# erizmr/SPH_Taichi

Hardware: AMD Instinct MI355X
Metric: WCSPH steps/sec at 1.74 M particles (+ ms/step breakdown sort/neighbour/force) (higher is better)
Workload: dtype f32

## Files before the change

### include/sph_hip.h

```cpp
#ifndef SPH_HIP_H
#define SPH_HIP_H

#include <stddef.h>
#include <stdint.h>

#ifdef __cplusplus
extern "C" {
#endif

#define SPH_ABI_VERSION 6

typedef struct SphContext SphContext;

typedef struct SphParams {
    int32_t n_particles;
    int32_t capacity;
    int32_t grid_num[3];
    int32_t cell_origin[3];
    int32_t n_objects;
    int32_t cold_capacity;
    float grid_size;
    float support_radius;
    float particle_diameter;
    float m_V0;
    float density_0;
    float stiffness;
    float exponent;
    float viscosity;
    float surface_tension;
    float dt;
    float g[3];
    float domain_size[3];
    float padding;
    float wall_hi[3];
    float k_w;
    float k_dw;
    float visc_d_nu;
    float visc_eps;
} SphParams;

enum SphField {
    SPH_F_OBJECT_ID = 0,
    SPH_F_X = 1,
    SPH_F_X_0 = 2,
    SPH_F_V = 3,
    SPH_F_ACCELERATION = 4,
    SPH_F_M_V = 5,
    SPH_F_M = 6,
    SPH_F_DENSITY = 7,
    SPH_F_PRESSURE = 8,
    SPH_F_MATERIAL = 9,
    SPH_F_COLOR = 10,
    SPH_F_IS_DYNAMIC = 11,
    SPH_F_GRID_IDS = 12,
    SPH_F_GRID_PARTICLES_NUM = 13,
    SPH_F_PID = 14,
    SPH_F_RIGID_REST_CM = 15,
    SPH_F_DFSPH_FACTOR = 16,
    SPH_F_DENSITY_ADV = 17,
    SPH_F_COUNT_ = 18
};

enum SphError {
    SPH_OK = 0,
    SPH_E_INVALID = -1,
    SPH_E_NO_DEVICE = -2,
    SPH_E_NOMEM = -3,
    SPH_E_STATE = -4
};

enum SphOption {
    SPH_OPT_GATHER_IMPL = 0,
    SPH_OPT_TIMING = 1,
    SPH_OPT_FUSED_STEP = 2,
    SPH_OPT_BRICK_SHAPE = 3,
    SPH_OPT_NO_DYNAMIC_SOLIDS = 4 ,
    SPH_OPT_DEBUG_ABLATE = 5,
    SPH_OPT_SLAB_DROP_OUTSIDE = 6 ,
    SPH_OPT_UNIFORM_FLUID = 7  ,
    SPH_OPT_UNIFORM_FLUID_STATE = 8 ,
    SPH_OPT_SORT_BY_PID = 9    ,
    SPH_OPT_KERNEL_VARIANT = 10 ,
    SPH_OPT_RIGID_BATCH = 11   ,
    SPH_OPT_DF_RUNAHEAD = 13,
    SPH_OPT_EXACT_MATH = 12    ,
    SPH_OPT_RIGID_SUMS_FROM_X0 = 14,
    SPH_OPT_PURE_FLUID_INSTANCE = 15 ,
    SPH_OPT_BRICK_RECORDS = 16 ,
    SPH_OPT_DF_FUSE_ERROR = 17
};
#define SPH_VAR_GROUPS 1
#define SPH_VAR_MFMA 32
#define SPH_VAR_GAT_LDS 2
#define SPH_VAR_GAT_LDS4 4
#define SPH_VAR_FORCE_BF 8
#define SPH_VAR_DEEP 16

typedef struct SphTimings {
    double sort_ms, neighbour_ms, force_ms, integrate_ms, halo_ms, total_ms;
    int64_t steps;
} SphTimings;

int32_t sph_abi_version(void);
int32_t sph_device_count(void);

int32_t sph_create(const SphParams* params, int32_t device, void* stream, SphContext** out);
int32_t sph_destroy(SphContext* ctx);
const char* sph_last_error(const SphContext* ctx);
int32_t sph_set_option(SphContext* ctx, int32_t option, int32_t value);
int32_t sph_get_option(const SphContext* ctx, int32_t option, int32_t* value);
int32_t sph_set_params(SphContext* ctx, const SphParams* params);
int32_t sph_set_dt(SphContext* ctx, float dt);
int32_t sph_set_particle_count(SphContext* ctx, int32_t n);

int32_t sph_upload(SphContext* ctx, int32_t field, const void* host, size_t bytes);
int32_t sph_download(SphContext* ctx, int32_t field, void* host, size_t bytes);

int32_t sph_update_grid_id(SphContext* ctx);
int32_t sph_prefix_sum(SphContext* ctx);
int32_t sph_counting_sort(SphContext* ctx);
int32_t sph_initialize_particle_system(SphContext* ctx);

int32_t sph_compute_boundary_volume(SphContext* ctx, int32_t dynamic);
int32_t sph_compute_densities(SphContext* ctx);
int32_t sph_compute_non_pressure_forces(SphContext* ctx);
int32_t sph_compute_pressure_forces(SphContext* ctx);
int32_t sph_advect(SphContext* ctx);
int32_t sph_enforce_boundary_3D(SphContext* ctx, int32_t particle_type);
int32_t sph_compute_rigid_rest_cm(SphContext* ctx, int32_t object_id);
int32_t sph_solve_constraints(SphContext* ctx, int32_t object_id, float* R_out);
int32_t sph_compute_com(SphContext* ctx, int32_t object_id, float* cm_out);

int32_t sph_step(SphContext* ctx, int32_t n_steps, const int32_t* dynamic_ids, int32_t n_dynamic);

int32_t sph_sync(SphContext* ctx);
int32_t sph_get_timings(SphContext* ctx, SphTimings* out);
int32_t sph_reset_timings(SphContext* ctx);

typedef struct SphStats {
    int64_t targets;
    int64_t list_entries;
    int32_t max_list;
    int32_t list_overflow_targets;
    int32_t lds_overflow_targets;
    int32_t max_cell_occupancy;
    int32_t nonempty_cells;
    int32_t polar_fallbacks;
} SphStats;
int32_t sph_get_stats(SphContext* ctx, SphStats* out);

#define SPH_RECORD_BYTES 48
int32_t sph_get_particle_count(SphContext* ctx, int32_t* n);
int32_t sph_layer_offsets(SphContext* ctx, const int32_t* layers, int32_t n, int32_t* out);
int32_t sph_layer_offsets_begin(SphContext* ctx, const int32_t* layers, int32_t n);
int32_t sph_layer_offsets_end(SphContext* ctx, int32_t* out, int32_t n);
int32_t sph_select_range(SphContext* ctx, int32_t first, int32_t count);
int32_t sph_truncate(SphContext* ctx, int32_t n);
int32_t sph_pack_range(SphContext* ctx, int32_t first, int32_t count, void* device_dst);
int32_t sph_append_records(SphContext* ctx, const void* device_src, int32_t count);
int32_t sph_set_target_layers(SphContext* ctx, int32_t density_lo, int32_t density_hi, int32_t force_lo, int32_t force_hi);
int32_t sph_slab_set_window(SphContext* ctx, int32_t origin_x, int32_t nx);
int32_t sph_slab_pack(SphContext* ctx, int32_t firstL, int32_t nL, void* dstL, int32_t firstR, int32_t nR, void* dstR);
int32_t sph_slab_advance(SphContext* ctx, int32_t keep_first, int32_t keep_count, const void* srcL, int32_t nL,
                         const void* srcR, int32_t nR, const int32_t* layers, int32_t n_layers, int32_t do_sweeps);
int32_t sph_slab_forces(SphContext* ctx, int32_t bl_lo, int32_t bl_hi, int32_t br_lo, int32_t br_hi,
                        int32_t firstL, int32_t nL, void* dstL, int32_t firstR, int32_t nR, void* dstR);
int32_t sph_slab_wait_pack(SphContext* ctx);
int32_t sph_slab_density(SphContext* ctx);
int32_t sph_sort(SphContext* ctx);
int32_t sph_sweeps(SphContext* ctx);

int32_t sph_rigid_partial_sums(SphContext* ctx, int32_t object_id, int32_t first, int32_t count, double* dev_sums16);
int32_t sph_rigid_apply_sums(SphContext* ctx, int32_t object_id, const double* dev_sums16, int32_t mode);
int32_t sph_upload_rest_positions(SphContext* ctx, const int32_t* pid, const float* x0, int32_t n);

typedef struct SphComm SphComm;
const char* sph_comm_last_error(void);
int32_t sph_comm_available(void);
int32_t sph_comm_unique_id(uint8_t* out128);
int32_t sph_comm_create(SphContext* ctx, const uint8_t* id128, int32_t rank, int32_t world, SphComm** out);
int32_t sph_comm_destroy(SphComm* comm);
int32_t sph_slab_announce(SphContext* ctx, SphComm* comm, int32_t left, int32_t right, int32_t n_to_left, int32_t n_to_right);
int32_t sph_slab_incoming(SphContext* ctx, SphComm* comm, int32_t* n_from_left, int32_t* n_from_right);
int32_t sph_slab_exchange(SphContext* ctx, SphComm* comm, int32_t left, int32_t right, const void* send_left, int32_t n_to_left,
                          const void* send_right, int32_t n_to_right, void* recv_left, int32_t n_from_left, void* recv_right,
                          int32_t n_from_right, int32_t after_packers);
int32_t sph_comm_swap(SphContext* ctx, SphComm* comm, int32_t left, int32_t right, const void* send_left, int64_t bytes_to_left,
                      const void* send_right, int64_t bytes_to_right, void* recv_left, int64_t bytes_from_left, void* recv_right,
                      int64_t bytes_from_right);
int32_t sph_comm_all_reduce(SphContext* ctx, SphComm* comm, void* dev, int32_t n, int32_t dtype);
int32_t sph_comm_sync(SphContext* ctx, SphComm* comm);
int32_t sph_comm_halo_time(SphContext* ctx, SphComm* comm, double* ms, int64_t* exchanges);
int32_t sph_comm_info(SphContext* ctx, SphComm* comm, int32_t* rank, int32_t* world);

typedef struct SphDfsphParams {
    int32_t enable_divergence_solver;
    int32_t m_max_iterations_v;
    int32_t m_max_iterations;
    int32_t fluid_particle_num;
    float m_eps;
    float reserved_;
    double max_error_V;
    double max_error;
} SphDfsphParams;

typedef struct SphDfsphStats {
    int32_t iterations_v;
    int32_t iterations;
    double avg_density_err_v;
    double avg_density_err;
    int64_t total_iterations_v;
    int64_t total_iterations;
    int64_t steps;
} SphDfsphStats;

int32_t sph_dfsph_set_params(SphContext* ctx, const SphDfsphParams* params);
int32_t sph_dfsph_get_stats(SphContext* ctx, SphDfsphStats* out);
int32_t sph_dfsph_compute_densities(SphContext* ctx);
int32_t sph_dfsph_compute_DFSPH_factor(SphContext* ctx);
int32_t sph_dfsph_compute_density_change(SphContext* ctx);
int32_t sph_dfsph_compute_density_adv(SphContext* ctx);
int32_t sph_dfsph_compute_density_error(SphContext* ctx, float offset, float* out);
int32_t sph_dfsph_multiply_time_step(SphContext* ctx, float time_step);
int32_t sph_dfsph_divergence_solver_iteration_kernel(SphContext* ctx);
int32_t sph_dfsph_pressure_solve_iteration_kernel(SphContext* ctx);
int32_t sph_dfsph_divergence_solve(SphContext* ctx);
int32_t sph_dfsph_pressure_solve(SphContext* ctx);
int32_t sph_dfsph_compute_non_pressure_forces(SphContext* ctx);
int32_t sph_dfsph_predict_velocity(SphContext* ctx);
int32_t sph_dfsph_advect(SphContext* ctx);
int32_t sph_dfsph_step(SphContext* ctx, int32_t n_steps, const int32_t* dynamic_ids, int32_t n_dynamic);
int32_t sph_dfsph_compute_density_error_range(SphContext* ctx, float offset, int32_t first, int32_t count, double* out);
int32_t sph_copy_velocity_records(SphContext* ctx, int32_t first, int32_t count, void* device_buf, int32_t to_context);

#define SPH_RENDER_MAX_INVISIBLE 32
typedef struct SphRenderParams {
    int32_t width, height;
    float eye[3], lookat[3], up[3];
    float fov_y_deg;
    float radius;
    float near_plane;
    float light[3];
    float ambient;
    uint8_t background[3], draw_box;
    float box_end[3];
    float box_color[3];
} SphRenderParams;
int32_t sph_render_set_params(SphContext* ctx, const SphRenderParams* params);
int32_t sph_render_set_invisible(SphContext* ctx, const int32_t* object_ids, int32_t n);
int32_t sph_render_frame(SphContext* ctx);
int32_t sph_render_download(SphContext* ctx, uint8_t* rgb, size_t bytes);
int32_t sph_render_download_depth(SphContext* ctx, float* depth, size_t bytes);

#define SPH_MAX_KINEMATIC 8
typedef struct SphKinematicMotion {
    int32_t object_id;
    float pivot[3];
    double lin_vel[3], ang_vel[3], osc_amplitude[3], osc_frequency, osc_phase, start_time, end_time;
} SphKinematicMotion;
typedef struct SphBodyPose {
    int32_t object_id;
    float R[9];
    float pivot[3], origin[3], lin_vel[3], ang_vel[3];
} SphBodyPose;
int32_t sph_kinematic_set(SphContext* ctx, const SphKinematicMotion* motions, int32_t n);
int32_t sph_kinematic_apply(SphContext* ctx, const SphBodyPose* poses, int32_t n);
int32_t sph_get_time(SphContext* ctx, double* t);
int32_t sph_set_time(SphContext* ctx, double t);

#define SPH_DIAG_BLOCKS 1024
#define SPH_DIAG_THREADS 256
#define SPH_DIAG_MAX_OBJECTS 96
typedef struct SphDiagRow {
    int64_t count;
    int64_t fluid_count;
    int64_t moving_count;
    double mass;
    double mx[3];
    double momentum[3];
    double kinetic;
    double v2_max;
    double a2_max;
    float density_min, density_max, pressure_min, pressure_max;
    float lo[3], hi[3];
} SphDiagRow;
int32_t sph_diag_reduce(SphContext* ctx);
int32_t sph_diag_download(SphContext* ctx, SphDiagRow* rows, int32_t n_rows);

#define SPH_COLUMNS_MAX (1 << 20)
#define SPH_COLUMNS_V_SCALE_LOG2 20
typedef struct SphColumnParams {
    int32_t axis;
    int32_t n[2];
    float origin[2], inv_cell[2];
    int32_t object_id;
} SphColumnParams;
typedef struct SphColumnTotals { int64_t selected, binned, outside; } SphColumnTotals;
int32_t sph_columns_reduce(SphContext* ctx, const SphColumnParams* params);
int32_t sph_columns_download(SphContext* ctx, int64_t* count, int64_t* sum_v , float* top, float* bottom,
                             int32_t n_columns, SphColumnTotals* totals);

#define SPH_EXPORT_X        1
#define SPH_EXPORT_V        2
#define SPH_EXPORT_DENSITY  4
#define SPH_EXPORT_PRESSURE 8
#define SPH_EXPORT_MASS     16
#define SPH_EXPORT_ID       32
#define SPH_EXPORT_OBJECT   64
#define SPH_EXPORT_MAX_OBJECTS 32
typedef struct SphExportParams {
    int32_t fields;
    int32_t material;
    int32_t n_objects;
    int32_t object_ids[SPH_EXPORT_MAX_OBJECTS];
    int32_t pid_stride, pid_phase;
    int32_t use_box;
    float box_lo[3], box_hi[3];
} SphExportParams;
typedef struct SphExportInfo { int64_t selected, rows; int32_t row_bytes, duplicate_ids; } SphExportInfo;
int32_t sph_export_select(SphContext* ctx, const SphExportParams* params);
int32_t sph_export_info(SphContext* ctx, SphExportInfo* info);
int32_t sph_export_download(SphContext* ctx, void* host, size_t bytes);

#define SPH_SURFACE_MAX_FILTER_R 16
#define SPH_SURFACE_MAX_ITERATIONS 8
#define SPH_SURFACE_PASSES 6
typedef struct SphSurfaceParams {
    int32_t iterations;
    float filter_radius;
    float depth_range;
    float fluid_color[3];
    float absorb[3];
    float sky[3];
    float f0;
    float specular;
} SphSurfaceParams;
int32_t sph_surface_set_params(SphContext* ctx, const SphSurfaceParams* params);
int32_t sph_surface_frame(SphContext* ctx);
int32_t sph_surface_download(SphContext* ctx, uint8_t* rgb, size_t bytes);
int32_t sph_surface_download_depth(SphContext* ctx, float* depth, size_t bytes);
int32_t sph_surface_download_thickness(SphContext* ctx, float* thickness, size_t bytes);
int32_t sph_surface_frame_timed(SphContext* ctx, float* ms, int32_t n);

#define SPH_FIELD_MAX_OBJECTS 32
enum SphColourField { SPH_FIELD_SPEED = 0, SPH_FIELD_VX, SPH_FIELD_VY, SPH_FIELD_VZ, SPH_FIELD_DENSITY, SPH_FIELD_PRESSURE,
                      SPH_FIELD_X, SPH_FIELD_Y, SPH_FIELD_Z, SPH_FIELD_COUNT_ };
typedef struct SphFieldColour {
    int32_t field;
    int32_t material;
    int32_t n_objects;
    int32_t object_ids[SPH_FIELD_MAX_OBJECTS];
    float lo, hi;
    float axis_origin;
} SphFieldColour;
typedef struct SphFieldRange { float lo, hi; int64_t count, non_finite; } SphFieldRange;
int32_t sph_frame_set_colour(SphContext* ctx, const SphFieldColour* colour, const int32_t* lut);
int32_t sph_field_range(SphContext* ctx, const SphFieldColour* colour, SphFieldRange* out);
int32_t sph_frame_download_field_index(SphContext* ctx, int32_t* index, size_t bytes);

#ifdef __cplusplus
}
#endif
#endif
```

### sph_taichi_amd/_lib.py

```python
from __future__ import annotations

import ctypes as C
import os

from . import build as _build

_F3 = C.c_float * 3
_I3 = C.c_int32 * 3


class SphParams(C.Structure):
    _fields_ = [
        ("n_particles", C.c_int32), ("capacity", C.c_int32), ("grid_num", _I3), ("cell_origin", _I3),
        ("n_objects", C.c_int32), ("cold_capacity", C.c_int32),
        ("grid_size", C.c_float), ("support_radius", C.c_float), ("particle_diameter", C.c_float),
        ("m_V0", C.c_float), ("density_0", C.c_float), ("stiffness", C.c_float), ("exponent", C.c_float),
        ("viscosity", C.c_float), ("surface_tension", C.c_float), ("dt", C.c_float),
        ("g", _F3), ("domain_size", _F3), ("padding", C.c_float), ("wall_hi", _F3),
        ("k_w", C.c_float), ("k_dw", C.c_float), ("visc_d_nu", C.c_float), ("visc_eps", C.c_float),
    ]


class SphTimings(C.Structure):
    _fields_ = [("sort_ms", C.c_double), ("neighbour_ms", C.c_double), ("force_ms", C.c_double),
                ("integrate_ms", C.c_double), ("halo_ms", C.c_double), ("total_ms", C.c_double),
                ("steps", C.c_int64)]


class SphStats(C.Structure):
    _fields_ = [("targets", C.c_int64), ("list_entries", C.c_int64), ("max_list", C.c_int32),
                ("list_overflow_targets", C.c_int32), ("lds_overflow_targets", C.c_int32),
                ("max_cell_occupancy", C.c_int32), ("nonempty_cells", C.c_int32), ("polar_fallbacks", C.c_int32)]


class SphDfsphParams(C.Structure):
    _fields_ = [("enable_divergence_solver", C.c_int32), ("m_max_iterations_v", C.c_int32),
                ("m_max_iterations", C.c_int32), ("fluid_particle_num", C.c_int32), ("m_eps", C.c_float),
                ("reserved_", C.c_float), ("max_error_V", C.c_double), ("max_error", C.c_double)]


class SphDfsphStats(C.Structure):
    _fields_ = [("iterations_v", C.c_int32), ("iterations", C.c_int32), ("avg_density_err_v", C.c_double),
                ("avg_density_err", C.c_double), ("total_iterations_v", C.c_int64), ("total_iterations", C.c_int64),
                ("steps", C.c_int64)]


class SphRenderParams(C.Structure):
    _fields_ = [("width", C.c_int32), ("height", C.c_int32), ("eye", _F3), ("lookat", _F3), ("up", _F3),
                ("fov_y_deg", C.c_float), ("radius", C.c_float), ("near_plane", C.c_float), ("light", _F3),
                ("ambient", C.c_float), ("background", C.c_uint8 * 3), ("draw_box", C.c_uint8),
                ("box_end", _F3), ("box_color", _F3)]


RENDER_MAX_INVISIBLE = 32
_D3 = C.c_double * 3


class SphKinematicMotion(C.Structure):
    _fields_ = [("object_id", C.c_int32), ("pivot", _F3), ("lin_vel", _D3), ("ang_vel", _D3), ("osc_amplitude", _D3),
                ("osc_frequency", C.c_double), ("osc_phase", C.c_double), ("start_time", C.c_double), ("end_time", C.c_double)]


class SphBodyPose(C.Structure):
    _fields_ = [("object_id", C.c_int32), ("R", C.c_float * 9), ("pivot", _F3), ("origin", _F3), ("lin_vel", _F3),
                ("ang_vel", _F3)]


MAX_KINEMATIC = 8


class SphDiagRow(C.Structure):
    _fields_ = [("count", C.c_int64), ("fluid_count", C.c_int64), ("moving_count", C.c_int64), ("mass", C.c_double),
                ("mx", _D3), ("momentum", _D3), ("kinetic", C.c_double), ("v2_max", C.c_double), ("a2_max", C.c_double),
                ("density_min", C.c_float), ("density_max", C.c_float), ("pressure_min", C.c_float),
                ("pressure_max", C.c_float), ("lo", _F3), ("hi", _F3)]


DIAG_BLOCKS, DIAG_THREADS, DIAG_MAX_OBJECTS = 1024, 256, 96

class SphColumnParams(C.Structure):
    _fields_ = [("axis", C.c_int32), ("n", C.c_int32 * 2), ("origin", C.c_float * 2), ("inv_cell", C.c_float * 2),
                ("object_id", C.c_int32)]


class SphColumnTotals(C.Structure):
    _fields_ = [("selected", C.c_int64), ("binned", C.c_int64), ("outside", C.c_int64)]


COLUMNS_MAX, COLUMNS_V_SCALE_LOG2 = 1 << 20, 20

class SphExportParams(C.Structure):
    _fields_ = [("fields", C.c_int32), ("material", C.c_int32), ("n_objects", C.c_int32), ("object_ids", C.c_int32 * 32),
                ("pid_stride", C.c_int32), ("pid_phase", C.c_int32), ("use_box", C.c_int32), ("box_lo", _F3), ("box_hi", _F3)]


class SphExportInfo(C.Structure):
    _fields_ = [("selected", C.c_int64), ("rows", C.c_int64), ("row_bytes", C.c_int32), ("duplicate_ids", C.c_int32)]


EXPORT_X, EXPORT_V, EXPORT_DENSITY, EXPORT_PRESSURE, EXPORT_MASS, EXPORT_ID, EXPORT_OBJECT = 1, 2, 4, 8, 16, 32, 64
EXPORT_MAX_OBJECTS = 32

class SphSurfaceParams(C.Structure):
    _fields_ = [("iterations", C.c_int32), ("filter_radius", C.c_float), ("depth_range", C.c_float), ("fluid_color", _F3),
                ("absorb", _F3), ("sky", _F3), ("f0", C.c_float), ("specular", C.c_float)]


SURFACE_MAX_FILTER_R, SURFACE_MAX_ITERATIONS, SURFACE_PASSES = 16, 8, 6
SURFACE_PASS_NAMES = ("clear", "opaque_splat", "fluid_splat", "depth_smoothing", "thickness_smoothing", "shade_resolve")

FIELD_MAX_OBJECTS = 32


class SphFieldColour(C.Structure):
    _fields_ = [("field", C.c_int32), ("material", C.c_int32), ("n_objects", C.c_int32), ("object_ids", C.c_int32 * FIELD_MAX_OBJECTS),
                ("lo", C.c_float), ("hi", C.c_float), ("axis_origin", C.c_float)]


class SphFieldRange(C.Structure):
    _fields_ = [("lo", C.c_float), ("hi", C.c_float), ("count", C.c_int64), ("non_finite", C.c_int64)]


F_OBJECT_ID, F_X, F_X_0, F_V, F_ACCELERATION, F_M_V, F_M, F_DENSITY, F_PRESSURE, F_MATERIAL, F_COLOR, \
    F_IS_DYNAMIC, F_GRID_IDS, F_GRID_PARTICLES_NUM, F_PID, F_RIGID_REST_CM, F_DFSPH_FACTOR, F_DENSITY_ADV = range(18)
OPT_GATHER_IMPL, OPT_TIMING, OPT_FUSED_STEP, OPT_BRICK_SHAPE, OPT_NO_DYNAMIC_SOLIDS, OPT_DEBUG_ABLATE, \
    OPT_SLAB_DROP_OUTSIDE, OPT_UNIFORM_FLUID, OPT_UNIFORM_FLUID_STATE, OPT_SORT_BY_PID, OPT_KERNEL_VARIANT, \
    OPT_RIGID_BATCH, OPT_EXACT_MATH, OPT_DF_RUNAHEAD, OPT_RIGID_SUMS_FROM_X0, OPT_PURE_FLUID_INSTANCE, OPT_BRICK_RECORDS, OPT_DF_FUSE_ERROR = range(18)
VAR_GROUPS, VAR_GAT_LDS, VAR_GAT_LDS4, VAR_FORCE_BF, VAR_DEEP, VAR_MFMA = 1, 2, 4, 8, 16, 32
VAR_DEFAULT = VAR_GROUPS | VAR_FORCE_BF | VAR_DEEP

ABI_VERSION = 6

_ctx = C.c_void_p
SYMBOLS = [
    ("sph_abi_version", C.c_int32, []),
    ("sph_device_count", C.c_int32, []),
    ("sph_create", C.c_int32, [C.POINTER(SphParams), C.c_int32, C.c_void_p, C.POINTER(_ctx)]),
    ("sph_destroy", C.c_int32, [_ctx]),
    ("sph_last_error", C.c_char_p, [_ctx]),
    ("sph_set_option", C.c_int32, [_ctx, C.c_int32, C.c_int32]),
    ("sph_get_option", C.c_int32, [_ctx, C.c_int32, C.POINTER(C.c_int32)]),
    ("sph_set_params", C.c_int32, [_ctx, C.POINTER(SphParams)]),
    ("sph_set_dt", C.c_int32, [_ctx, C.c_float]),
    ("sph_set_particle_count", C.c_int32, [_ctx, C.c_int32]),
    ("sph_upload", C.c_int32, [_ctx, C.c_int32, C.c_void_p, C.c_size_t]),
    ("sph_download", C.c_int32, [_ctx, C.c_int32, C.c_void_p, C.c_size_t]),
    ("sph_update_grid_id", C.c_int32, [_ctx]),
    ("sph_prefix_sum", C.c_int32, [_ctx]),
    ("sph_counting_sort", C.c_int32, [_ctx]),
    ("sph_initialize_particle_system", C.c_int32, [_ctx]),
    ("sph_compute_boundary_volume", C.c_int32, [_ctx, C.c_int32]),
    ("sph_compute_densities", C.c_int32, [_ctx]),
    ("sph_compute_non_pressure_forces", C.c_int32, [_ctx]),
    ("sph_compute_pressure_forces", C.c_int32, [_ctx]),
    ("sph_advect", C.c_int32, [_ctx]),
    ("sph_enforce_boundary_3D", C.c_int32, [_ctx, C.c_int32]),
    ("sph_compute_rigid_rest_cm", C.c_int32, [_ctx, C.c_int32]),
    ("sph_solve_constraints", C.c_int32, [_ctx, C.c_int32, C.POINTER(C.c_float)]),
    ("sph_compute_com", C.c_int32, [_ctx, C.c_int32, C.POINTER(C.c_float)]),
    ("sph_step", C.c_int32, [_ctx, C.c_int32, C.POINTER(C.c_int32), C.c_int32]),
    ("sph_sync", C.c_int32, [_ctx]),
    ("sph_get_timings", C.c_int32, [_ctx, C.POINTER(SphTimings)]),
    ("sph_reset_timings", C.c_int32, [_ctx]),
    ("sph_get_stats", C.c_int32, [_ctx, C.POINTER(SphStats)]),
    ("sph_get_particle_count", C.c_int32, [_ctx, C.POINTER(C.c_int32)]),
    ("sph_layer_offsets", C.c_int32, [_ctx, C.POINTER(C.c_int32), C.c_int32, C.POINTER(C.c_int32)]),
    ("sph_layer_offsets_begin", C.c_int32, [_ctx, C.POINTER(C.c_int32), C.c_int32]),
    ("sph_layer_offsets_end", C.c_int32, [_ctx, C.POINTER(C.c_int32), C.c_int32]),
    ("sph_select_range", C.c_int32, [_ctx, C.c_int32, C.c_int32]),
    ("sph_truncate", C.c_int32, [_ctx, C.c_int32]),
    ("sph_pack_range", C.c_int32, [_ctx, C.c_int32, C.c_int32, C.c_void_p]),
    ("sph_append_records", C.c_int32, [_ctx, C.c_void_p, C.c_int32]),
    ("sph_set_target_layers", C.c_int32, [_ctx, C.c_int32, C.c_int32, C.c_int32, C.c_int32]),
    ("sph_slab_set_window", C.c_int32, [_ctx, C.c_int32, C.c_int32]),
    ("sph_slab_pack", C.c_int32, [_ctx, C.c_int32, C.c_int32, C.c_void_p, C.c_int32, C.c_int32, C.c_void_p]),
    ("sph_slab_advance", C.c_int32, [_ctx, C.c_int32, C.c_int32, C.c_void_p, C.c_int32, C.c_void_p, C.c_int32,
                                     C.POINTER(C.c_int32), C.c_int32, C.c_int32]),
    ("sph_slab_forces", C.c_int32, [_ctx, C.c_int32, C.c_int32, C.c_int32, C.c_int32, C.c_int32, C.c_int32, C.c_void_p,
                                    C.c_int32, C.c_int32, C.c_void_p]),
    ("sph_slab_wait_pack", C.c_int32, [_ctx]),
    ("sph_slab_density", C.c_int32, [_ctx]),
    ("sph_sort", C.c_int32, [_ctx]),
    ("sph_sweeps", C.c_int32, [_ctx]),
    ("sph_rigid_partial_sums", C.c_int32, [_ctx, C.c_int32, C.c_int32, C.c_int32, C.c_void_p]),
    ("sph_rigid_apply_sums", C.c_int32, [_ctx, C.c_int32, C.c_void_p, C.c_int32]),
    ("sph_upload_rest_positions", C.c_int32, [_ctx, C.c_void_p, C.c_void_p, C.c_int32]),
    ("sph_dfsph_set_params", C.c_int32, [_ctx, C.POINTER(SphDfsphParams)]),
    ("sph_dfsph_get_stats", C.c_int32, [_ctx, C.POINTER(SphDfsphStats)]),
    ("sph_dfsph_compute_densities", C.c_int32, [_ctx]),
    ("sph_dfsph_compute_DFSPH_factor", C.c_int32, [_ctx]),
    ("sph_dfsph_compute_density_change", C.c_int32, [_ctx]),
    ("sph_dfsph_compute_density_adv", C.c_int32, [_ctx]),
    ("sph_dfsph_compute_density_error", C.c_int32, [_ctx, C.c_float, C.POINTER(C.c_float)]),
    ("sph_dfsph_multiply_time_step", C.c_int32, [_ctx, C.c_float]),
    ("sph_dfsph_divergence_solver_iteration_kernel", C.c_int32, [_ctx]),
    ("sph_dfsph_pressure_solve_iteration_kernel", C.c_int32, [_ctx]),
    ("sph_dfsph_divergence_solve", C.c_int32, [_ctx]),
    ("sph_dfsph_pressure_solve", C.c_int32, [_ctx]),
    ("sph_dfsph_compute_non_pressure_forces", C.c_int32, [_ctx]),
    ("sph_dfsph_predict_velocity", C.c_int32, [_ctx]),
    ("sph_dfsph_advect", C.c_int32, [_ctx]),
    ("sph_dfsph_step", C.c_int32, [_ctx, C.c_int32, C.POINTER(C.c_int32), C.c_int32]),
    ("sph_dfsph_compute_density_error_range", C.c_int32, [_ctx, C.c_float, C.c_int32, C.c_int32, C.POINTER(C.c_double)]),
    ("sph_copy_velocity_records", C.c_int32, [_ctx, C.c_int32, C.c_int32, C.c_void_p, C.c_int32]),
    ("sph_comm_last_error", C.c_char_p, []),
    ("sph_comm_available", C.c_int32, []),
    ("sph_comm_unique_id", C.c_int32, [C.c_void_p]),
    ("sph_comm_create", C.c_int32, [_ctx, C.c_void_p, C.c_int32, C.c_int32, C.POINTER(C.c_void_p)]),
    ("sph_comm_destroy", C.c_int32, [C.c_void_p]),
    ("sph_slab_announce", C.c_int32, [_ctx, C.c_void_p, C.c_int32, C.c_int32, C.c_int32, C.c_int32]),
    ("sph_slab_incoming", C.c_int32, [_ctx, C.c_void_p, C.POINTER(C.c_int32), C.POINTER(C.c_int32)]),
    ("sph_slab_exchange", C.c_int32, [_ctx, C.c_void_p, C.c_int32, C.c_int32, C.c_void_p, C.c_int32, C.c_void_p, C.c_int32,
                                      C.c_void_p, C.c_int32, C.c_void_p, C.c_int32, C.c_int32]),
    ("sph_comm_swap", C.c_int32, [_ctx, C.c_void_p, C.c_int32, C.c_int32, C.c_void_p, C.c_int64, C.c_void_p, C.c_int64,
                                  C.c_void_p, C.c_int64, C.c_void_p, C.c_int64]),
    ("sph_comm_all_reduce", C.c_int32, [_ctx, C.c_void_p, C.c_void_p, C.c_int32, C.c_int32]),
    ("sph_comm_sync", C.c_int32, [_ctx, C.c_void_p]),
    ("sph_comm_halo_time", C.c_int32, [_ctx, C.c_void_p, C.POINTER(C.c_double), C.POINTER(C.c_int64)]),
    ("sph_comm_info", C.c_int32, [_ctx, C.c_void_p, C.POINTER(C.c_int32), C.POINTER(C.c_int32)]),
    ("sph_render_set_params", C.c_int32, [_ctx, C.POINTER(SphRenderParams)]),
    ("sph_render_set_invisible", C.c_int32, [_ctx, C.POINTER(C.c_int32), C.c_int32]),
    ("sph_render_frame", C.c_int32, [_ctx]),
    ("sph_render_download", C.c_int32, [_ctx, C.c_void_p, C.c_size_t]),
    ("sph_render_download_depth", C.c_int32, [_ctx, C.c_void_p, C.c_size_t]),
    ("sph_kinematic_set", C.c_int32, [_ctx, C.POINTER(SphKinematicMotion), C.c_int32]),
    ("sph_kinematic_apply", C.c_int32, [_ctx, C.POINTER(SphBodyPose), C.c_int32]),
    ("sph_get_time", C.c_int32, [_ctx, C.POINTER(C.c_double)]),
    ("sph_set_time", C.c_int32, [_ctx, C.c_double]),
    ("sph_diag_reduce", C.c_int32, [_ctx]),
    ("sph_diag_download", C.c_int32, [_ctx, C.POINTER(SphDiagRow), C.c_int32]),
    ("sph_columns_reduce", C.c_int32, [_ctx, C.POINTER(SphColumnParams)]),
    ("sph_columns_download", C.c_int32, [_ctx, C.c_void_p, C.c_void_p, C.c_void_p, C.c_void_p, C.c_int32,
                                         C.POINTER(SphColumnTotals)]),
    ("sph_export_select", C.c_int32, [_ctx, C.POINTER(SphExportParams)]),
    ("sph_export_info", C.c_int32, [_ctx, C.POINTER(SphExportInfo)]),
    ("sph_export_download", C.c_int32, [_ctx, C.c_void_p, C.c_size_t]),
    ("sph_surface_set_params", C.c_int32, [_ctx, C.POINTER(SphSurfaceParams)]),
    ("sph_surface_frame", C.c_int32, [_ctx]),
    ("sph_surface_download", C.c_int32, [_ctx, C.c_void_p, C.c_size_t]),
    ("sph_surface_download_depth", C.c_int32, [_ctx, C.c_void_p, C.c_size_t]),
    ("sph_surface_download_thickness", C.c_int32, [_ctx, C.c_void_p, C.c_size_t]),
    ("sph_surface_frame_timed", C.c_int32, [_ctx, C.POINTER(C.c_float), C.c_int32]),
    ("sph_frame_set_colour", C.c_int32, [_ctx, C.POINTER(SphFieldColour), C.c_void_p]),
    ("sph_field_range", C.c_int32, [_ctx, C.POINTER(SphFieldColour), C.POINTER(SphFieldRange)]),
    ("sph_frame_download_field_index", C.c_int32, [_ctx, C.c_void_p, C.c_size_t]),
]

_LIB = None


class SphError(RuntimeError):
    pass


def profiling_variant() -> bool:
    return os.environ.get("SPH_HIP_LIB_VARIANT", "") == "profile"


def experiment_variant() -> str:
    v = os.environ.get("SPH_HIP_LIB_VARIANT", "")
    return v if v.startswith("x-") else ""


def library_path() -> str:
    if experiment_variant():
        return os.path.join(os.path.dirname(_build.LIB), f"libsph_hip_{experiment_variant()}.so")
    return _build.LIB_PROFILE if profiling_variant() else _build.LIB


def _preload_shared_hip_runtime():
    import importlib.util
    try:
        spec = importlib.util.find_spec("torch")
    except (ImportError, ValueError):
        spec = None
    if spec is None or not spec.origin:
        return
    cand = os.path.join(os.path.dirname(spec.origin), "lib", "libamdhip64.so")
    if os.path.exists(cand):
        try:
            C.CDLL(cand, mode=C.RTLD_GLOBAL)
        except OSError:
            pass


def load(build_if_missing: bool = True):
    global _LIB
    if _LIB is not None:
        return _LIB
    path = library_path()
    if build_if_missing and not experiment_variant() and _build.stale(profiling_variant()):
        try:
            _build.build(profile=profiling_variant())
        except Exception as e:
            if not os.path.exists(path):
                raise SphError(f"libsph_hip.so is missing and could not be built: {e}") from e
    if not os.path.exists(path):
        raise SphError(f"{path} not found: run `python -m sph_taichi_amd.build` (needs hipcc)")
    _preload_shared_hip_runtime()
    lib = C.CDLL(path)
    for name, res, args in SYMBOLS:
        fn = getattr(lib, name)
        fn.restype = res
        fn.argtypes = args
    if lib.sph_abi_version() != ABI_VERSION:
        raise SphError(f"libsph_hip ABI {lib.sph_abi_version()} != binding {ABI_VERSION}")
    _LIB = lib
    return lib


def check(lib, ctx, rc: int, what: str):
    if rc != 0:
        msg = lib.sph_last_error(ctx)
        raise SphError(f"{what} failed (rc={rc}): {msg.decode() if msg else ''}")
```

### sph_taichi_amd/csrc/sph_api.hip

```cpp
#include <math.h>
#include <sched.h>
#include <new>
#include <vector>
#include "sph_internal.h"

#define SCAN_TILE 2048

int sphk_init_pid(SphContext* c);
int sphk_build_dyn_list(SphContext* c);

static thread_local char g_err[256] = "";

int sph_fail(SphContext* c, int code, const char* what) {
    if (c) snprintf(c->err, sizeof(c->err), "%s", what);
    else snprintf(g_err, sizeof(g_err), "%s", what);
    return code;
}

DevView sph_view(const SphContext* c) {
    DevView d;
    const SphParams& p = c->p;
    d.N = c->N; d.G = c->G;
    d.nx = p.grid_num[0]; d.ny = p.grid_num[1]; d.nz = p.grid_num[2];
    d.tgt_lo = 0; d.tgt_hi = p.grid_num[0]; d.tgt_lo2 = d.tgt_hi2 = 0;
#ifdef SPH_PROFILE
    d.ablate = c->opt_ablate;
    d.prof_ts = (c->opt_ablate & (3 << 28)) ? reinterpret_cast<unsigned long long*>(c->stage) : nullptr;
#endif
    d.drop_outside = c->opt_drop_outside;
    d.sort_by_pid = c->opt_sort_by_pid;
    d.ox = p.cell_origin[0]; d.oy = p.cell_origin[1]; d.oz = p.cell_origin[2];
    d.grid_size = p.grid_size; d.h = p.support_radius; d.inv_h = 1.0f / p.support_radius;
    d.d2 = p.particle_diameter * p.particle_diameter;
    d.m_V0 = p.m_V0; d.rho0 = p.density_0; d.stiffness = p.stiffness; d.exponent = p.exponent;
    d.exp_int = (p.exponent >= 1.0f && p.exponent <= 32.0f && p.exponent == (float)(int)p.exponent) ? (int)p.exponent : 0;
    d.sigma = p.surface_tension; d.dt = p.dt;
    d.gx = p.g[0]; d.gy = p.g[1]; d.gz = p.g[2];
    d.pad = p.padding;
    d.k_w = p.k_w; d.k_dw = p.k_dw; d.visc_d_nu = p.visc_d_nu; d.visc_eps = p.visc_eps;
    d.w_zero = p.k_w * (6.0f * 0.0f - 6.0f * 0.0f + 1.0f);
    {
        const float q = p.particle_diameter / p.support_radius;
        if (q <= 0.5f) d.w_d = p.k_w * (6.0f * q * q * q - 6.0f * q * q + 1.0f);
        else if (q <= 1.0f) d.w_d = p.k_w * 2.0f * (1.0f - q) * (1.0f - q) * (1.0f - q);
        else d.w_d = 0.0f;
    }
    const int o = c->in_off;
    d.xm = c->xm[c->cur] + o; d.vf = c->vf[c->cur] + o; d.aux = c->aux[c->cur] + o; d.key = c->key[c->cur] + o;
    d.eos = c->eos; d.eos2 = reinterpret_cast<float2*>(c->eos); d.acc = c->acc + o; d.acc_fx = c->acc_fx + 3 * (size_t)o; d.cell_end = c->cell_end;
    d.x0_cold = c->x0_cold; d.rigid_rest_cm = c->rigid_rest_cm; d.polar_fb = c->dyn_count ? c->dyn_count + 3 : nullptr;
    d.m_eps = c->df.m_eps;
    d.stg = c->stg; d.gat = c->gat; d.kbuf = reinterpret_cast<float*>(c->gat);
    d.m_u = c->m_uniform; d.write_sg = 0; d.write_k = 0;
    d.whx = p.wall_hi[0]; d.why = p.wall_hi[1]; d.whz = p.wall_hi[2];
    d.fuse_advect = 0; d.store_acc = 1; d.df_bpart = nullptr;
    d.gate = (c->df_epoch && c->opt_df_runahead) ? c->df_gate : nullptr;
    d.gate_epoch = c->df_epoch;
    d.fx_scale = ldexp(1.0, c->rigid_fx_exp);
    d.rigid_from_x0 = 0;
    return d;
}

__global__ void k_read_layer_offsets(const int* __restrict__ cell_end, const int* __restrict__ layers, int n,
                                     int per_layer, int* __restrict__ out) {
    const int k = blockIdx.x * blockDim.x + threadIdx.x;
    if (k >= n) return;
    const int L = layers[k];
    out[k] = L > 0 ? cell_end[(size_t)L * per_layer - 1] : 0;
}

__global__ void k_read_cells(const int* __restrict__ cell_end, CellIdx16 ix, int* __restrict__ out) {
    const int k = threadIdx.x;
    if (k < 16 && ix.v[k] >= 0) out[k] = cell_end[ix.v[k]];
}

int sph_check_device_flags(SphContext* c) {
    if (c->h_pinned && ((volatile int*)c->h_pinned)[16]) {
        ((volatile int*)c->h_pinned)[16] = 0;
        c->sorted = c->have_prefix = c->have_keys = false;
        sph_invalidate_lists(c);
        return sph_fail(c, SPH_E_STATE, "prefix sum: a scan tile never saw a predecessor's total (k_scan_fused's bounded wait ran out); "
                                        "the cell table of that sort and every result since are invalid: re-upload the state and sort again");
    }
    return 0;
}

static bool variant_mask_ok(int v) { return (v & (SPH_VAR_GAT_LDS | SPH_VAR_GAT_LDS4)) != (SPH_VAR_GAT_LDS | SPH_VAR_GAT_LDS4); }

struct KinPose64 { double R[9], c[3], u[3], w[3]; };
static void kin_pose(const SphKinematicMotion& m, double t, KinPose64* out) {
    const double tc = t < m.start_time ? m.start_time : (t > m.end_time ? m.end_time : t);
    const double tau = tc - m.start_time;
    const bool active = t >= m.start_time && t <= m.end_time;
    const double two_pi = 6.283185307179586476925286766559;
    const double arg = two_pi * m.osc_frequency * tau + m.osc_phase;
    const double s = sin(arg) - sin(m.osc_phase), ds = two_pi * m.osc_frequency * cos(arg);
    for (int a = 0; a < 3; ++a) {
        out->c[a] = (double)m.pivot[a] + (m.lin_vel[a] * tau + m.osc_amplitude[a] * s);
        out->u[a] = active ? m.lin_vel[a] + m.osc_amplitude[a] * ds : 0.0;
        out->w[a] = active ? m.ang_vel[a] : 0.0;
    }
    const double wn = sqrt(m.ang_vel[0] * m.ang_vel[0] + m.ang_vel[1] * m.ang_vel[1] + m.ang_vel[2] * m.ang_vel[2]);
    double* R = out->R;
    for (int k = 0; k < 9; ++k) R[k] = (k % 4 == 0) ? 1.0 : 0.0;
    if (wn > 0.0) {
        const double k[3] = {m.ang_vel[0] / wn, m.ang_vel[1] / wn, m.ang_vel[2] / wn};
        const double th = wn * tau, sn = sin(th), cs1 = 1.0 - cos(th);
        const double K[9] = {0.0, -k[2], k[1], k[2], 0.0, -k[0], -k[1], k[0], 0.0};
        for (int i = 0; i < 3; ++i)
            for (int j = 0; j < 3; ++j) {
                double kk = 0.0;
                for (int l = 0; l < 3; ++l) kk += K[3 * i + l] * K[3 * l + j];
                R[3 * i + j] += sn * K[3 * i + j] + cs1 * kk;
            }
    }
}

static int sph_obj_info(SphContext* c) {
    if (c->obj_info_valid) return 0;
    const int no = c->p.n_objects;
    if (!c->obj_info) {
        c->obj_info = new (std::nothrow) SphContext::ObjInfo[no > 0 ? no : 1];
        if (!c->obj_info) return sph_fail(c, SPH_E_NOMEM, "kinematic bodies: out of host memory");
    }
    for (int o = 0; o < no; ++o) {
        c->obj_info[o].n = c->obj_info[o].n_static = 0;
        for (int a = 0; a < 3; ++a) { c->obj_info[o].lo[a] = INFINITY; c->obj_info[o].hi[a] = -INFINITY; }
    }
    if (c->N > 0) {
        std::vector<float> rec;
        try { rec.resize((size_t)c->N * 4); } catch (...) { return sph_fail(c, SPH_E_NOMEM, "kinematic bodies: out of host memory"); }
        int rc = sphk_rest_records(c, reinterpret_cast<float4*>(c->stage));
        if (rc) return rc;
        SPH_HIP(c, hipMemcpyAsync(rec.data(), c->stage, rec.size() * sizeof(float), hipMemcpyDeviceToHost, c->stream));
        SPH_HIP(c, hipStreamSynchronize(c->stream));
        for (int i = 0; i < c->N; ++i) {
            int fl;
            memcpy(&fl, &rec[4 * (size_t)i + 3], sizeof(int));
            const int o = (int)((unsigned)fl >> 9);
            if (o >= no) continue;
            SphContext::ObjInfo& I = c->obj_info[o];
            I.n += 1;
            I.n_static += (fl & 0x1FF) == 0 ? 1 : 0;
            for (int a = 0; a < 3; ++a) {
                const double v = (double)rec[4 * (size_t)i + a];
                I.lo[a] = v < I.lo[a] ? v : I.lo[a];
                I.hi[a] = v > I.hi[a] ? v : I.hi[a];
            }
        }
    }
    c->obj_info_valid = true;
    return 0;
}

static int kin_check_object(SphContext* c, const char* who, int object_id) {
    if (object_id < 0 || object_id >= c->p.n_objects) {
        snprintf(c->err, sizeof(c->err), "%s: object id %d is outside [0, n_objects = %d)", who, object_id, c->p.n_objects);
        return SPH_E_INVALID;
    }
    const SphContext::ObjInfo& I = c->obj_info[object_id];
    if (I.n == 0) {
        snprintf(c->err, sizeof(c->err), "%s: object %d has no particles", who, object_id);
        return SPH_E_INVALID;
    }
    if (I.n_static != I.n) {
        snprintf(c->err, sizeof(c->err), "%s: object %d has %d dynamic or fluid particles: only a non-dynamic solid can be kinematic", who,
                 object_id, I.n - I.n_static);
        return SPH_E_INVALID;
    }
    return 0;
}

static bool kin_contained(const SphContext* c, int object_id, const double R[9], const double pivot[3], const double origin[3]) {
    const SphContext::ObjInfo& I = c->obj_info[object_id];
    for (int k = 0; k < 8; ++k) {
        const double q[3] = {((k & 1) ? I.hi[0] : I.lo[0]) - pivot[0], ((k & 2) ? I.hi[1] : I.lo[1]) - pivot[1],
                             ((k & 4) ? I.hi[2] : I.lo[2]) - pivot[2]};
        for (int a = 0; a < 3; ++a) {
            const double x = origin[a] + (R[3 * a] * q[0] + R[3 * a + 1] * q[1] + R[3 * a + 2] * q[2]);
            if (!(x >= (double)c->p.padding && x <= (double)c->p.domain_size[a] - (double)c->p.padding)) return false;
        }
    }
    return true;
}

static void kin_poses_at(const SphContext* c, double t, KinPoses* P) {
    P->n = c->n_kin;
    for (int k = 0; k < SPH_MAX_KINEMATIC; ++k) P->id[k] = -1;
    for (int k = 0; k < c->n_kin; ++k) {
        const SphKinematicMotion& m = c->kin[k];
        KinPose64 q;
        kin_pose(m, t, &q);
        P->id[k] = m.object_id;
        for (int j = 0; j < 9; ++j) P->R[k][j] = (float)q.R[j];
        for (int a = 0; a < 3; ++a) {
            P->pivot[k][a] = m.pivot[a];
            P->origin[k][a] = (float)q.c[a];
            P->lin[k][a] = (float)q.u[a];
            P->ang[k][a] = (float)q.w[a];
        }
    }
}

static int kin_admit(SphContext* c, int n_steps, int* n_run) {
    *n_run = 0;
    if (!c->obj_info_valid) {
        int rc = sph_obj_info(c);
        for (int k = 0; k < c->n_kin && !rc; ++k) rc = kin_check_object(c, "kinematic step", c->kin[k].object_id);
        if (rc) return rc;
    }
    double t = c->sim_time;
    for (int it = 0; it < n_steps; ++it) {
        t += (double)c->p.dt;
        for (int k = 0; k < c->n_kin; ++k) {
            const SphKinematicMotion& m = c->kin[k];
            KinPose64 q;
            kin_pose(m, t, &q);
            const double pivot[3] = {(double)m.pivot[0], (double)m.pivot[1], (double)m.pivot[2]};
            if (!kin_contained(c, m.object_id, q.R, pivot, q.c)) {
                snprintf(c->err, sizeof(c->err), "kinematic object %d would leave [padding, domain - padding] at the end of step %d of this call "
                         "(t = %.9g): that step and the later ones were not enqueued, %d step(s) were", m.object_id, it, t, it);
                *n_run = it;
                return SPH_E_INVALID;
            }
        }
    }
    *n_run = n_steps;
    return 0;
}

extern "C" {

int32_t sph_abi_version(void) { return SPH_ABI_VERSION; }

int32_t sph_device_count(void) {
    int n = 0;
    if (hipGetDeviceCount(&n) != hipSuccess) return 0;
    return n;
}

const char* sph_last_error(const SphContext* ctx) { return ctx ? ctx->err : g_err; }

static int alloc_dev(SphContext* c, void** p, size_t bytes) {
    hipError_t e = hipMalloc(p, bytes ? bytes : 16);
    if (e != hipSuccess) {
        snprintf(c->err, sizeof(c->err), "hipMalloc(%zu) failed: %s", bytes, hipGetErrorString(e));
        return SPH_E_NOMEM;
    }
    e = hipMemsetAsync(*p, 0, bytes ? bytes : 16, c->stream);
    return e == hipSuccess ? 0 : (int)e;
}

int32_t sph_create(const SphParams* params, int32_t device, void* stream, SphContext** out) {
    if (!params || !out) return sph_fail(nullptr, SPH_E_INVALID, "sph_create: null argument");
    *out = nullptr;
    int ndev = 0;
    if (hipGetDeviceCount(&ndev) != hipSuccess || ndev <= 0)
        return sph_fail(nullptr, SPH_E_NO_DEVICE, "sph_create: no HIP device visible (libsph_hip needs an MI355X/gfx950 GPU)");
    if (device < 0 || device >= ndev) return sph_fail(nullptr, SPH_E_INVALID, "sph_create: bad device index");
    if (params->n_particles < 0 || params->capacity < params->n_particles || params->grid_num[0] <= 0 ||
        params->grid_num[1] <= 0 || params->grid_num[2] <= 0 || params->n_objects < 0)
        return sph_fail(nullptr, SPH_E_INVALID, "sph_create: bad sizes");
    if ((long long)params->grid_num[0] * params->grid_num[1] * params->grid_num[2] > 0x7ffff000LL)
        return sph_fail(nullptr, SPH_E_INVALID, "sph_create: grid too large for i32 cell ids");
    if (hipSetDevice(device) != hipSuccess) return sph_fail(nullptr, SPH_E_NO_DEVICE, "hipSetDevice failed");
    hipDeviceProp_t prop;
    if (hipGetDeviceProperties(&prop, device) == hipSuccess && strncmp(prop.gcnArchName, "gfx950", 6) != 0) {
        snprintf(g_err, sizeof(g_err), "sph_create: device arch %s is not gfx950", prop.gcnArchName);
        return SPH_E_NO_DEVICE;
    }
    SphContext* c = new SphContext();
    memset(c, 0, sizeof(*c));
    c->p = *params;
    c->device = device;
    c->N = params->n_particles;
    c->cap = params->capacity > 0 ? params->capacity : 1;
    c->G = params->grid_num[0] * params->grid_num[1] * params->grid_num[2];
    c->nx_alloc = params->grid_num[0];
    c->tgt_layers[0] = c->tgt_layers[2] = 0;
    c->tgt_layers[1] = c->tgt_layers[3] = params->grid_num[0];
    c->opt_gather_impl = 1;
    c->opt_fused = 1;
    c->opt_timing = 0;
    c->timing_phase = 0;
    c->opt_brick_shape = 0;
    c->opt_rigid_batch = 1;
    c->opt_df_fuse_err = 1;
    c->opt_df_runahead = 0;
    c->opt_exact_math = 0;
    c->opt_rigid_x0 = 0;
    c->opt_pure_instance = 1;
    c->opt_brick_rec = 1;
    if (stream) { c->stream = (hipStream_t)stream; c->own_stream = false; }
    else {
        if (hipStreamCreateWithFlags(&c->stream, hipStreamNonBlocking) != hipSuccess) {
            delete c;
            return sph_fail(nullptr, SPH_E_NO_DEVICE, "hipStreamCreate failed");
        }
        c->own_stream = true;
    }
    const size_t cap = (size_t)c->cap;
    c->scan_blocks = (c->G + 1 + SCAN_TILE - 1) / SCAN_TILE;
    int rc = 0;
    for (int s = 0; s < 2 && !rc; ++s) {
        rc = rc ? rc : alloc_dev(c, (void**)&c->xm[s], cap * 16);
        rc = rc ? rc : alloc_dev(c, (void**)&c->vf[s], cap * 16);
        rc = rc ? rc : alloc_dev(c, (void**)&c->aux[s], cap * 16);
        rc = rc ? rc : alloc_dev(c, (void**)&c->key[s], cap * 4);
    }
    rc = rc ? rc : alloc_dev(c, (void**)&c->eos, cap * 16);
    rc = rc ? rc : alloc_dev(c, (void**)&c->stg, cap * 16);
    rc = rc ? rc : alloc_dev(c, (void**)&c->gat, cap * 16);
    rc = rc ? rc : alloc_dev(c, (void**)&c->acc, cap * 16);
    rc = rc ? rc : alloc_dev(c, (void**)&c->acc_tmp, cap * 16);
    rc = rc ? rc : alloc_dev(c, (void**)&c->acc_fx, cap * 3 * sizeof(long long));
    rc = rc ? rc : alloc_dev(c, (void**)&c->cell_buf[0], (size_t)c->scan_blocks * SCAN_TILE * 4);
    rc = rc ? rc : alloc_dev(c, (void**)&c->cell_buf[1], (size_t)c->scan_blocks * SCAN_TILE * 4);
    if (!rc) { c->cell_cur = 0; c->cell_end = c->cell_buf[0]; c->next_cells_zero = false; }
    rc = rc ? rc : alloc_dev(c, (void**)&c->rank_off, cap * 4);
    rc = rc ? rc : alloc_dev(c, (void**)&c->idx_unstable, cap * 4);
    rc = rc ? rc : alloc_dev(c, (void**)&c->scan_status, (size_t)(c->scan_blocks + 1) * 8);
    {
        int sh = 3;
        while (((size_t)1 << sh) < cap * 8) ++sh;
        const bool reach = (((unsigned long long)(SPH_GLIST_ROWS / 4 + 4)) << sh) <= (1ull << 32);
        c->glist_shift = reach ? sh : 0;
        rc = rc ? rc : alloc_dev(c, (void**)&c->glist, reach ? ((size_t)(SPH_GLIST_ROWS / 4) << sh) : 16);
    }
    rc = rc ? rc : alloc_dev(c, (void**)&c->gcnt, cap);
    c->brick_cap = ((params->grid_num[0] + 3) / 4) * ((params->grid_num[1] + 1) / 2) * params->grid_num[2] + 8;
    rc = rc ? rc : alloc_dev(c, (void**)&c->brick_list, (size_t)c->brick_cap * 8);
    rc = rc ? rc : alloc_dev(c, (void**)&c->brick_count, 16);
    rc = rc ? rc : alloc_dev(c, (void**)&c->brick_rec, (size_t)c->brick_cap * 32 * sizeof(int4));
    rc = rc ? rc : alloc_dev(c, (void**)&c->brick_list2, (size_t)c->brick_cap * 8);
    rc = rc ? rc : alloc_dev(c, (void**)&c->brick_count2, 16);
    const size_t cold = params->cold_capacity > 0 ? (size_t)params->cold_capacity : cap;
    if (cold < cap) { sph_destroy(c); return sph_fail(nullptr, SPH_E_INVALID, "sph_create: cold_capacity < capacity"); }
    c->cold_cap = (int)cold;
    rc = rc ? rc : alloc_dev(c, (void**)&c->x0_cold, cold * 12);
    rc = rc ? rc : alloc_dev(c, (void**)&c->color_cold, cold * 12);
    rc = rc ? rc : alloc_dev(c, (void**)&c->rigid_rest_cm, (size_t)(params->n_objects > 0 ? params->n_objects : 1) * 12);
    rc = rc ? rc : alloc_dev(c, (void**)&c->dyn_list, cap * 4);
    rc = rc ? rc : alloc_dev(c, (void**)&c->dyn_count, 16);
    c->rigid_part_blocks = (c->cap + 255) / 256 + 1;
    rc = rc ? rc : alloc_dev(c, (void**)&c->rigid_part, (size_t)c->rigid_part_blocks * 16 * sizeof(double));
    rc = rc ? rc : alloc_dev(c, (void**)&c->rigid_R, 16 * sizeof(float));
    rc = rc ? rc : alloc_dev(c, (void**)&c->df_err, sizeof(double));
    rc = rc ? rc : alloc_dev(c, (void**)&c->df_part, SPH_DF_ERR_BLOCKS * sizeof(double));
    rc = rc ? rc : alloc_dev(c, (void**)&c->df_bpart, (size_t)c->brick_cap * sizeof(double));
    if (!rc && hipHostMalloc((void**)&c->h_df_err, sizeof(double), hipHostMallocMapped) != hipSuccess) rc = SPH_E_NOMEM;
    if (!rc && hipHostMalloc((void**)&c->h_df_slot, 4 * sizeof(*c->h_df_slot), hipHostMallocMapped) != hipSuccess) rc = SPH_E_NOMEM;
    rc = rc ? rc : alloc_dev(c, (void**)&c->df_gate, 16);
    for (int k = 0; k < 4 && !rc; ++k)
        if (hipEventCreateWithFlags(&c->ev_df[k], hipEventDisableTiming) != hipSuccess) rc = SPH_E_NOMEM;
    c->stage_bytes = cap * 16 > (size_t)c->G * 4 ? cap * 16 : (size_t)c->G * 4;
    if (c->stage_bytes < 65536) c->stage_bytes = 65536;
    rc = rc ? rc : alloc_dev(c, &c->stage, c->stage_bytes);
    if (!rc && hipHostMalloc((void**)&c->h_pinned, 32 * sizeof(int), hipHostMallocMapped) != hipSuccess) rc = SPH_E_NOMEM;
    if (!rc) {
        memset(c->h_pinned, 0, 32 * sizeof(int));
        int* dev = nullptr;
        if (hipHostGetDevicePointer((void**)&dev, c->h_pinned, 0) != hipSuccess) rc = SPH_E_NOMEM;
        else c->scan_err = dev + 16;
    }
    if (!rc && hipEventCreateWithFlags(&c->ev_off, hipEventDisableTiming) != hipSuccess) rc = SPH_E_NOMEM;
    if (!rc && hipEventCreateWithFlags(&c->ev_pack, hipEventDisableTiming) != hipSuccess) rc = SPH_E_NOMEM;
    if (!rc && hipEventCreateWithFlags(&c->ev_fork, hipEventDisableTiming) != hipSuccess) rc = SPH_E_NOMEM;
    if (!rc && hipStreamCreateWithFlags(&c->side, hipStreamNonBlocking) != hipSuccess) rc = SPH_E_NOMEM;
    if (!rc) rc = sphk_init_pid(c);
    for (int s = 0; s < SPH_MAX_TIMED_STEPS && !rc; ++s)
        for (int k = 0; k < 5 && !rc; ++k)
            if (hipEventCreate(&c->ev[s][k]) != hipSuccess) rc = SPH_E_NOMEM;
    if (!rc && hipStreamSynchronize(c->stream) != hipSuccess) rc = SPH_E_NO_DEVICE;
    if (rc) {
        snprintf(g_err, sizeof(g_err), "sph_create failed: %s", c->err);
        sph_destroy(c);
        return rc;
    }
    c->n_dyn_host = -1;
    c->rigid_fx_exp = 30;
    sph_invalidate_lists(c);
    c->opt_uniform = -1; c->uniform_state = -1; c->m_uniform = 0.0f;
    c->opt_variant = SPH_VAR_DEFAULT;
    if (const char* e = getenv("SPH_KERNEL_VARIANT")) { const int v = atoi(e) & 31; c->opt_variant = variant_mask_ok(v) ? v : SPH_VAR_DEFAULT; }
    memset(&c->df_stats, 0, sizeof(c->df_stats));
    c->df.enable_divergence_solver = 1; c->df.m_max_iterations_v = 100; c->df.m_max_iterations = 100;
    c->df.fluid_particle_num = 0; c->df.m_eps = 1e-5f; c->df.reserved_ = 0.0f; c->df.max_error_V = 0.1; c->df.max_error = 0.05;
    *out = c;
    return 0;
}

int32_t sph_destroy(SphContext* c) {
    if (!c) return 0;
    (void)hipSetDevice(c->device);
    if (c->stream) (void)hipStreamSynchronize(c->stream);
    void* ptrs[] = {c->xm[0], c->xm[1], c->vf[0], c->vf[1], c->aux[0], c->aux[1], c->key[0], c->key[1], c->eos, c->stg, c->gat, c->acc,
                    c->acc_tmp, c->cell_buf[0], c->cell_buf[1], c->rank_off, c->idx_unstable, c->scan_status, c->x0_cold, c->color_cold,
                    c->rigid_rest_cm, c->dyn_list, c->dyn_count, c->acc_fx, c->rigid_part, c->rigid_R, c->df_err, c->df_part, c->df_bpart, c->stage, c->glist, c->gcnt, c->brick_list, c->brick_count, c->brick_list2, c->brick_count2, c->brick_rec};
    for (void* p : ptrs) if (p) (void)hipFree(p);
    sph_render_release(c);
    sph_diag_release(c);
    sph_columns_release(c);
    sph_export_release(c);
    sph_surface_release(c);
    delete[] c->obj_info;
    for (int s = 0; s < SPH_MAX_TIMED_STEPS; ++s)
        for (int k = 0; k < 5; ++k) if (c->ev[s][k]) (void)hipEventDestroy(c->ev[s][k]);
    if (c->h_pinned) (void)hipHostFree(c->h_pinned);
    if (c->h_df_err) (void)hipHostFree(c->h_df_err);
    if (c->h_df_slot) (void)hipHostFree(c->h_df_slot);
    if (c->df_gate) (void)hipFree(c->df_gate);
    for (int k = 0; k < 4; ++k) if (c->ev_df[k]) (void)hipEventDestroy(c->ev_df[k]);
    if (c->ev_off) (void)hipEventDestroy(c->ev_off);
    if (c->ev_pack) (void)hipEventDestroy(c->ev_pack);
    if (c->ev_fork) (void)hipEventDestroy(c->ev_fork);
    if (c->side) (void)hipStreamDestroy(c->side);
    if (c->own_stream && c->stream) (void)hipStreamDestroy(c->stream);
    delete c;
    return 0;
}

int32_t sph_set_option(SphContext* c, int32_t option, int32_t value) {
    if (!c) return SPH_E_INVALID;
    switch (option) {
        case SPH_OPT_GATHER_IMPL: if (value < 0 || value > 1) return sph_fail(c, SPH_E_INVALID, "gather impl must be 0 or 1"); c->opt_gather_impl = value; c->uniform_state = -1; return 0;
        case SPH_OPT_TIMING: c->opt_timing = value > 0 ? value : 0; c->timing_phase = 0; return 0;
        case SPH_OPT_FUSED_STEP: c->opt_fused = value ? 1 : 0; return 0;
        case SPH_OPT_BRICK_SHAPE: if (value < 0 || value > 1) return sph_fail(c, SPH_E_INVALID, "brick shape must be 0 (adaptive height) or 1 (fixed 4x2x4)"); c->opt_brick_shape = value; sph_invalidate_lists(c); return 0;
        case SPH_OPT_NO_DYNAMIC_SOLIDS: c->opt_no_dynamic = value ? 1 : 0; c->n_dyn_host = -1; c->uniform_state = -1; return 0;
        case SPH_OPT_DEBUG_ABLATE:
#ifndef SPH_PROFILE
            if (value != 0) return sph_fail(c, SPH_E_INVALID, "section ablation exists only in the profiling build (python -m sph_taichi_amd.build --profile; bench.py --ablate loads it)");
#endif
            c->opt_ablate = value;
            return 0;
        case SPH_OPT_SLAB_DROP_OUTSIDE: c->opt_drop_outside = value ? 1 : 0; c->uniform_state = -1; return 0;
        case SPH_OPT_SORT_BY_PID: c->opt_sort_by_pid = value ? 1 : 0; return 0;
        case SPH_OPT_RIGID_BATCH: c->opt_rigid_batch = value ? 1 : 0; return 0;
        case SPH_OPT_EXACT_MATH: c->opt_exact_math = value ? 1 : 0; sph_invalidate_lists(c); return 0;
        case SPH_OPT_DF_RUNAHEAD: c->opt_df_runahead = value ? 1 : 0; return 0;
        case SPH_OPT_KERNEL_VARIANT:
            if (value < -1 || value > 63 || (value > 0 && !variant_mask_ok(value))) return sph_fail(c, SPH_E_INVALID, "kernel variant must be -1 (default) or a mask of SPH_VAR_* (GAT_LDS and GAT_LDS4 exclude each other)");
            c->opt_variant = value < 0 ? SPH_VAR_DEFAULT : value;
            sph_invalidate_lists(c);
            return 0;
        case SPH_OPT_UNIFORM_FLUID: if (value < -1 || value > 1) return sph_fail(c, SPH_E_INVALID, "uniform-fluid option must be -1, 0 or 1"); c->opt_uniform = value; c->uniform_state = -1; return 0;
        case SPH_OPT_RIGID_SUMS_FROM_X0: c->opt_rigid_x0 = value ? 1 : 0; return 0;
        case SPH_OPT_PURE_FLUID_INSTANCE:
            if (value < 0 || value > 2) return sph_fail(c, SPH_E_INVALID, "pure-fluid instance option must be 0, 1 or 2");
            c->opt_pure_instance = value; sph_invalidate_lists(c); return 0;
        case SPH_OPT_BRICK_RECORDS: c->opt_brick_rec = value ? 1 : 0; sph_invalidate_lists(c); return 0;
        case SPH_OPT_DF_FUSE_ERROR: c->opt_df_fuse_err = value ? 1 : 0; return 0;
    }
    return sph_fail(c, SPH_E_INVALID, "unknown option");
}

int32_t sph_get_option(const SphContext* c, int32_t option, int32_t* value) {
    if (!c || !value) return SPH_E_INVALID;
    switch (option) {
        case SPH_OPT_GATHER_IMPL: *value = c->opt_gather_impl; return 0;
        case SPH_OPT_TIMING: *value = c->opt_timing; return 0;
        case SPH_OPT_FUSED_STEP: *value = c->opt_fused; return 0;
        case SPH_OPT_BRICK_SHAPE: *value = c->opt_brick_shape; return 0;
        case SPH_OPT_NO_DYNAMIC_SOLIDS: *value = c->opt_no_dynamic; return 0;
        case SPH_OPT_DEBUG_ABLATE: *value = c->opt_ablate; return 0;
        case SPH_OPT_SLAB_DROP_OUTSIDE: *value = c->opt_drop_outside; return 0;
        case SPH_OPT_UNIFORM_FLUID: *value = c->opt_uniform; return 0;
        case SPH_OPT_SORT_BY_PID: *value = c->opt_sort_by_pid; return 0;
        case SPH_OPT_RIGID_BATCH: *value = c->opt_rigid_batch; return 0;
        case SPH_OPT_EXACT_MATH: *value = (c->opt_exact_math && c->uniform_state != 0) ? 1 : 0; return 0;
        case SPH_OPT_KERNEL_VARIANT: *value = c->opt_variant; return 0;
        case SPH_OPT_DF_RUNAHEAD: *value = c->opt_df_runahead; return 0;
        case SPH_OPT_UNIFORM_FLUID_STATE: *value = c->uniform_state; return 0;
        case SPH_OPT_RIGID_SUMS_FROM_X0: *value = c->opt_rigid_x0; return 0;
        case SPH_OPT_PURE_FLUID_INSTANCE: *value = c->opt_pure_instance; return 0;
        case SPH_OPT_BRICK_RECORDS: *value = c->opt_brick_rec; return 0;
        case SPH_OPT_DF_FUSE_ERROR: *value = c->opt_df_fuse_err; return 0;
    }
    return SPH_E_INVALID;
}

int32_t sph_set_params(SphContext* c, const SphParams* p) {
    if (!c || !p) return SPH_E_INVALID;
    if (p->capacity != c->p.capacity || p->n_objects != c->p.n_objects || p->cold_capacity != c->p.cold_capacity ||
        memcmp(p->grid_num, c->p.grid_num, sizeof(p->grid_num)) != 0 ||
        memcmp(p->cell_origin, c->p.cell_origin, sizeof(p->cell_origin)) != 0)
        return sph_fail(c, SPH_E_INVALID, "sph_set_params: sizes differ from sph_create");
    const int n = c->p.n_particles;
    c->p = *p;
    c->p.n_particles = n;
    return 0;
}

int32_t sph_set_dt(SphContext* c, float dt) {
    if (!c) return SPH_E_INVALID;
    c->p.dt = dt;
    return 0;
}

int32_t sph_set_particle_count(SphContext* c, int32_t n) {
    if (!c || n < 0 || n > c->cap) return sph_fail(c, SPH_E_INVALID, "particle count out of range");
    c->N = n;
    c->n_dyn_host = -1;
    c->obj_info_valid = false;
    sph_forget_pure_fluid(c);
    sphd_set_changed(c->dv);
    c->have_keys = c->have_prefix = false;
    return 0;
}

static size_t field_bytes(const SphContext* c, int field) {
    switch (field) {
        case SPH_F_X: case SPH_F_X_0: case SPH_F_V: case SPH_F_ACCELERATION: case SPH_F_COLOR: return (size_t)c->N * 12;
        case SPH_F_GRID_PARTICLES_NUM: return (size_t)c->G * 4;
        case SPH_F_RIGID_REST_CM: return (size_t)c->p.n_objects * 12;
        default: return (size_t)c->N * 4;
    }
}

int32_t sph_upload(SphContext* c, int32_t field, const void* host, size_t bytes) {
    if (!c || !host) return SPH_E_INVALID;
    if (field < 0 || field >= SPH_F_COUNT_ || field == SPH_F_GRID_IDS || field == SPH_F_GRID_PARTICLES_NUM)
        return sph_fail(c, SPH_E_INVALID, "sph_upload: field is not uploadable");
    if (bytes != field_bytes(c, field)) return sph_fail(c, SPH_E_INVALID, "sph_upload: size mismatch");
    SPH_HIP(c, hipSetDevice(c->device));
    if (bytes == 0) return 0;
    if (field == SPH_F_DENSITY || field == SPH_F_PRESSURE) { int rc0 = sph_ensure_aux(c); if (rc0) return rc0; }
    if (field == SPH_F_ACCELERATION) c->acc_partial = false;
    if (field == SPH_F_RIGID_REST_CM) {
        SPH_HIP(c, hipMemcpyAsync(c->rigid_rest_cm, host, bytes, hipMemcpyHostToDevice, c->stream));
        SPH_HIP(c, hipStreamSynchronize(c->stream));
        return 0;
    }
    SPH_HIP(c, hipMemcpyAsync(c->stage, host, bytes, hipMemcpyHostToDevice, c->stream));
    int rc = sphk_insert(c, field, c->stage);
    if (rc) return rc;
    SPH_HIP(c, hipStreamSynchronize(c->stream));
    if (field == SPH_F_MATERIAL || field == SPH_F_IS_DYNAMIC || field == SPH_F_DENSITY) c->n_dyn_host = -1;
    if (field == SPH_F_MATERIAL || field == SPH_F_M || field == SPH_F_M_V) c->uniform_state = -1;
    if (field == SPH_F_X) c->have_keys = c->have_prefix = false;
    if (field == SPH_F_X_0 || field == SPH_F_OBJECT_ID || field == SPH_F_MATERIAL || field == SPH_F_IS_DYNAMIC || field == SPH_F_PID)
        c->obj_info_valid = false;
    return 0;
}

int32_t sph_download(SphContext* c, int32_t field, void* host, size_t bytes) {
    if (!c || !host) return SPH_E_INVALID;
    if (field < 0 || field >= SPH_F_COUNT_) return sph_fail(c, SPH_E_INVALID, "sph_download: bad field");
    if (bytes != field_bytes(c, field)) return sph_fail(c, SPH_E_INVALID, "sph_download: size mismatch");
    SPH_HIP(c, hipSetDevice(c->device));
    if (bytes == 0) return 0;
    if (field == SPH_F_ACCELERATION && c->acc_partial)
        return sph_fail(c, SPH_E_STATE, "sph_download(acceleration): the last sph_slab_forces consumed the interior particles' accelerations "
                                        "in its fused finish and did not write them out (stale values would be returned); call "
                                        "sph_compute_non_pressure_forces + sph_compute_pressure_forces, or run with SPH_OPT_FUSED_STEP 0");
    const void* src = c->stage;
    if (field == SPH_F_GRID_PARTICLES_NUM) src = c->cell_end;
    else if (field == SPH_F_RIGID_REST_CM) src = c->rigid_rest_cm;
    else {
        int rc = (field == SPH_F_DENSITY || field == SPH_F_PRESSURE) ? sph_ensure_aux(c) : 0;
        rc = rc ? rc : sphk_extract(c, field, c->stage);
        if (rc) return rc;
    }
    SPH_HIP(c, hipMemcpyAsync(host, src, bytes, hipMemcpyDeviceToHost, c->stream));
    SPH_HIP(c, hipStreamSynchronize(c->stream));
    return sph_check_device_flags(c);
}

static int refresh_dyn(SphContext* c) {
    if (c->n_dyn_host >= 0) return 0;
    if (c->opt_no_dynamic) { c->n_dyn_host = 0; return 0; }
    int rc = sphk_build_dyn_list(c);
    if (rc) return rc;
    int nr[2] = {0, 0};
    SPH_HIP(c, hipMemcpyAsync(nr, c->dyn_count, 2 * sizeof(int), hipMemcpyDeviceToHost, c->stream));
    SPH_HIP(c, hipStreamSynchronize(c->stream));
    c->n_dyn_host = nr[0];
    float rho_max;
    memcpy(&rho_max, &nr[1], sizeof(float));
    double L = 1.0;
    for (int a = 0; a < 3; ++a) L = fmax(L, 2.0 * fabs((double)c->p.domain_size[a]) + 1.0);
    const double bound = fmax((double)nr[0], 1.0) * fmax((double)c->p.m_V0 * fmax((double)rho_max, 1.0), 1e-30) * L * L;
    int e = 0;
    (void)frexp(bound, &e);
    c->rigid_fx_exp = 62 - e;
    if (c->rigid_fx_exp > 80) c->rigid_fx_exp = 80;
    if (c->rigid_fx_exp < -200) c->rigid_fx_exp = -200;
    return 0;
}

#define ENTER(c)                                  \
    if (!(c)) return SPH_E_INVALID;               \
    SPH_HIP((c), hipSetDevice((c)->device));

int32_t sph_update_grid_id(SphContext* c) {
    ENTER(c);
    int rc = sphk_hash_histogram(c);
    if (rc) return rc;
    c->have_keys = true;
    c->have_prefix = false;
    return 0;
}

int32_t sph_prefix_sum(SphContext* c) {
    ENTER(c);
    if (!c->have_keys) return sph_fail(c, SPH_E_STATE, "sph_prefix_sum before sph_update_grid_id");
    int rc = sphk_scan(c);
    if (rc) return rc;
    c->have_prefix = true;
    return 0;
}

static int counting_sort(SphContext* c, bool sort_acc, const CellIdx16* deliver_offsets = nullptr) {
    if (!c->have_prefix) return sph_fail(c, SPH_E_STATE, "sph_counting_sort before sph_prefix_sum");
    int rc = refresh_dyn(c);
    if (rc) return rc;
    rc = sphk_sort_scatter(c, sort_acc, deliver_offsets);
    if (rc) return rc;
    c->in_off = 0;
    c->have_keys = false;
    c->sorted = true;
    return 0;
}

int32_t sph_counting_sort(SphContext* c) {
    ENTER(c);
    int rc = sph_ensure_aux(c);
    return rc ? rc : counting_sort(c, true);
}

int32_t sph_initialize_particle_system(SphContext* c) {
    ENTER(c);
    int rc = sph_ensure_aux(c);
    rc = rc ? rc : sph_update_grid_id(c);
    rc = rc ? rc : sph_prefix_sum(c);
    rc = rc ? rc : counting_sort(c, true);
    return rc;
}

static int need_sorted(SphContext* c, const char* who) {
    if (!c->sorted || !c->have_prefix) {
        snprintf(c->err, sizeof(c->err), "%s needs the neighbour structure: call sph_initialize_particle_system first", who);
        return SPH_E_STATE;
    }
    return 0;
}

int32_t sph_compute_boundary_volume(SphContext* c, int32_t dynamic) {
    ENTER(c);
    int rc = need_sorted(c, "sph_compute_boundary_volume");
    rc = rc ? rc : refresh_dyn(c);
    return rc ? rc : sphk_gather(c, dynamic ? GM_BVOL_DYNAMIC : GM_BVOL_STATIC);
}

int32_t sph_compute_densities(SphContext* c) {
    ENTER(c);
    int rc = need_sorted(c, "sph_compute_densities");
    return rc ? rc : sphk_gather(c, GM_DENSITY);
}

int32_t sph_compute_non_pressure_forces(SphContext* c) {
    ENTER(c);
    int rc = need_sorted(c, "sph_compute_non_pressure_forces");
    rc = rc ? rc : sph_ensure_aux(c);
    rc = rc ? rc : sphk_gather(c, GM_NONPRESSURE);
    if (!rc) c->acc_partial = false;
    return rc;
}

int32_t sph_compute_pressure_forces(SphContext* c) {
    ENTER(c);
    int rc = need_sorted(c, "sph_compute_pressure_forces");
    rc = rc ? rc : sph_ensure_aux(c);
    rc = rc ? rc : sphk_eos(c);
    return rc ? rc : sphk_gather(c, GM_PRESSURE);
}

int32_t sph_advect(SphContext* c) {
    ENTER(c);
    return sphk_advect(c, false);
}

int32_t sph_enforce_boundary_3D(SphContext* c, int32_t particle_type) {
    ENTER(c);
    int rc = refresh_dyn(c);
    return rc ? rc : sphk_enforce_boundary(c, particle_type);
}

int32_t sph_compute_rigid_rest_cm(SphContext* c, int32_t object_id) {
    ENTER(c);
    if (object_id < 0 || object_id >= c->p.n_objects) return sph_fail(c, SPH_E_INVALID, "object id out of range");
    int rc = refresh_dyn(c);
    return rc ? rc : sphk_rigid_com(c, object_id, true);
}

int32_t sph_solve_constraints(SphContext* c, int32_t object_id, float* R_out) {
    ENTER(c);
    if (object_id < 0 || object_id >= c->p.n_objects) return sph_fail(c, SPH_E_INVALID, "object id out of range");
    int rc = refresh_dyn(c);
    rc = rc ? rc : sphk_rigid_solve(c, object_id);
    if (rc) return rc;
    if (R_out) {
        float tmp[12] = {0, 0, 0, 1, 0, 0, 0, 1, 0, 0, 0, 1};
        if (c->n_dyn_host > 0) {
            SPH_HIP(c, hipMemcpyAsync(tmp, c->rigid_R, sizeof(tmp), hipMemcpyDeviceToHost, c->stream));
            SPH_HIP(c, hipStreamSynchronize(c->stream));
        }
        memcpy(R_out, tmp + 3, 9 * sizeof(float));
    }
    return 0;
}

int32_t sph_compute_com(SphContext* c, int32_t object_id, float* cm_out) {
    ENTER(c);
    if (!cm_out) return SPH_E_INVALID;
    int rc = refresh_dyn(c);
    rc = rc ? rc : sphk_rigid_com(c, object_id, false);
    if (rc) return rc;
    SPH_HIP(c, hipMemcpyAsync(cm_out, c->rigid_R, 3 * sizeof(float), hipMemcpyDeviceToHost, c->stream));
    SPH_HIP(c, hipStreamSynchronize(c->stream));
    return 0;
}

static bool sph_timed_step(SphContext* c) {
    if (c->opt_timing <= 0) return false;
    const bool timed = c->timing_phase == 0;
    c->timing_phase = (c->timing_phase + 1) % c->opt_timing;
    return timed;
}

static int harvest_events(SphContext* c) {
    if (c->ev_used == 0) return 0;
    SPH_HIP(c, hipEventSynchronize(c->ev[c->ev_used - 1][4]));
    for (int s = 0; s < c->ev_used; ++s) {
        float ms[4];
        for (int k = 0; k < 4; ++k) SPH_HIP(c, hipEventElapsedTime(&ms[k], c->ev[s][k], c->ev[s][k + 1]));
        c->tm.sort_ms += ms[0];
        c->tm.neighbour_ms += ms[1];
        c->tm.force_ms += ms[2];
        c->tm.integrate_ms += ms[3];
        c->tm.total_ms += ms[0] + ms[1] + ms[2] + ms[3];
        c->tm.steps += 1;
    }
    c->ev_used = 0;
    return 0;
}

static int timed_step_begin(SphContext* c, hipEvent_t** ev) {
    *ev = nullptr;
    if (!sph_timed_step(c)) return 0;
    if (c->ev_used == SPH_MAX_TIMED_STEPS) { int rc = harvest_events(c); if (rc) return rc; }
    *ev = c->ev[c->ev_used];
    SPH_HIP(c, hipEventRecord((*ev)[0], c->stream));
    return 0;
}

static int uniform_fluid(SphContext* c) {
    if (c->opt_uniform == 0 || c->opt_gather_impl != 1 || (c->opt_drop_outside && !c->opt_no_dynamic)) {
        c->uniform_state = 0;
        return 0;
    }
    if (c->uniform_state >= 0) return 0;
    return sphk_check_uniform_fluid(c);
}

static int density_phase(SphContext* c) {
    int rc = c->n_dyn_host > 0 ? sphk_gather(c, GM_BVOL_DYNAMIC) : 0;
    rc = rc ? rc : uniform_fluid(c);
    return rc ? rc : sphk_gather(c, GM_DENSITY_EOS);
}

static int step_sweeps(SphContext* c, hipEvent_t* ev, const int32_t* dynamic_ids, int32_t n_dynamic, bool last_step) {
    int rc = 0;
    bool fused_advect = false;
    if (c->opt_fused) {
        rc = density_phase(c);
        if (rc) return rc;
        if (ev) SPH_HIP(c, hipEventRecord(ev[2], c->stream));
        const bool fuse = c->uniform_state == 1 && sphd_one_gather_wcsph(c->dv) && !c->opt_drop_outside &&
                          c->opt_gather_impl == 1 && c->N > 0;
        SweepArgs force;
        force.fuse_advect = fuse;
        force.store_acc = last_step;
        rc = sphk_gather(c, GM_FORCE_FUSED, force);
        if (rc) return rc;
        fused_advect = fuse;
    } else {
        rc = c->n_dyn_host > 0 ? sphk_gather(c, GM_BVOL_DYNAMIC) : 0;
        rc = rc ? rc : sphk_gather(c, GM_DENSITY);
        if (rc) return rc;
        if (ev) SPH_HIP(c, hipEventRecord(ev[2], c->stream));
        rc = sphk_gather(c, GM_NONPRESSURE);
        rc = rc ? rc : sphk_eos(c);
        rc = rc ? rc : sphk_gather(c, GM_PRESSURE);
        if (rc) return rc;
    }
    if (ev) SPH_HIP(c, hipEventRecord(ev[3], c->stream));
    if (fused_advect) return sphk_rigid_solve_all(c, dynamic_ids, n_dynamic, true);
    rc = sphk_advect(c, true);
    if (rc) return rc;
    if (c->n_dyn_host > 0) { rc = sphk_rigid_solve_all(c, dynamic_ids, n_dynamic, false); if (rc) return rc; }
    return 0;
}

static int sort_no_fold(SphContext* c, const CellIdx16* deliver_offsets = nullptr) {
    int rc = sph_update_grid_id(c);
    rc = rc ? rc : sph_prefix_sum(c);
    return rc ? rc : counting_sort(c, false, deliver_offsets);
}

int32_t sph_set_target_layers(SphContext* c, int32_t dlo, int32_t dhi, int32_t flo, int32_t fhi) {
    if (!c) return SPH_E_INVALID;
    const int nx = c->p.grid_num[0];
    if (dlo < 0 || dhi > nx || dlo > dhi || flo < 0 || fhi > nx || flo > fhi) return sph_fail(c, SPH_E_INVALID, "sph_set_target_layers: bad range");
    c->tgt_layers[0] = dlo; c->tgt_layers[1] = dhi; c->tgt_layers[2] = flo; c->tgt_layers[3] = fhi;
    return 0;
}

int32_t sph_slab_set_window(SphContext* c, int32_t origin_x, int32_t nx) {
    ENTER(c);
    if (nx <= 0 || nx > c->nx_alloc) return sph_fail(c, SPH_E_INVALID, "sph_slab_set_window: nx exceeds the allocation of sph_create");
    c->p.cell_origin[0] = origin_x;
    c->p.grid_num[0] = nx;
    c->G = nx * c->p.grid_num[1] * c->p.grid_num[2];
    c->scan_blocks = (c->G + 1 + SCAN_TILE - 1) / SCAN_TILE;
    c->tgt_layers[0] = c->tgt_layers[2] = 0;
    c->tgt_layers[1] = c->tgt_layers[3] = nx;
    c->next_cells_zero = false;
    sph_invalidate_lists(c);
    c->have_keys = c->have_prefix = c->sorted = false;
    c->n_dyn_host = -1;
    return 0;
}

int32_t sph_sort(SphContext* c) {
    ENTER(c);
    int rc = sph_ensure_aux(c);
    return rc ? rc : sort_no_fold(c);
}

int32_t sph_sweeps(SphContext* c) {
    ENTER(c);
    int rc = need_sorted(c, "sph_sweeps");
    rc = rc ? rc : refresh_dyn(c);
    if (rc) return rc;
    return step_sweeps(c, nullptr, nullptr, 0, true);
}

typedef int (*StepBody)(SphContext* c, hipEvent_t* ev, const int32_t* dynamic_ids, int32_t n_dynamic, bool last_step);

static int step_loop(SphContext* c, const char* who, StepBody body, int32_t n_steps, const int32_t* dynamic_ids, int32_t n_dynamic) {
    if (n_steps < 0 || n_dynamic < 0 || (n_dynamic > 0 && !dynamic_ids)) {
        snprintf(c->err, sizeof(c->err), "%s: bad arguments", who);
        return SPH_E_INVALID;
    }
    int rc = refresh_dyn(c);
    if (rc) return rc;
    int kin_rc = 0;
    if (c->n_kin > 0) {
        kin_rc = kin_admit(c, n_steps, &n_steps);
        if (kin_rc && kin_rc != SPH_E_INVALID) return kin_rc;
    }
    if (n_steps > 0) c->acc_partial = false;
    for (int it = 0; it < n_steps; ++it) {
        const double t_end = c->sim_time + (double)c->p.dt;
        hipEvent_t* ev = nullptr;
        rc = timed_step_begin(c, &ev);
        rc = rc ? rc : sort_no_fold(c);
        if (rc) return rc;
        if (ev) SPH_HIP(c, hipEventRecord(ev[1], c->stream));
        rc = body(c, ev, dynamic_ids, n_dynamic, it + 1 == n_steps);
        if (rc) return rc;
        if (c->n_kin > 0) {
            KinPoses kin;
            kin_poses_at(c, t_end, &kin);
            rc = sphk_kinematic_apply(c, kin);
            if (rc) return rc;
        }
        c->sim_time = t_end;
        if (ev) { SPH_HIP(c, hipEventRecord(ev[4], c->stream)); c->ev_used++; }
    }
    return kin_rc;
}

int32_t sph_step(SphContext* c, int32_t n_steps, const int32_t* dynamic_ids, int32_t n_dynamic) {
    ENTER(c);
    return step_loop(c, "sph_step", step_sweeps, n_steps, dynamic_ids, n_dynamic);
}

int32_t sph_get_particle_count(SphContext* c, int32_t* n) {
    if (!c || !n) return SPH_E_INVALID;
    *n = c->N;
    return 0;
}

int32_t sph_layer_offsets(SphContext* c, const int32_t* layers, int32_t n, int32_t* out) {
    ENTER(c);
    if (!layers || !out || n < 0) return SPH_E_INVALID;
    if (!c->have_prefix) return sph_fail(c, SPH_E_STATE, "sph_layer_offsets needs the prefix sum");
    const int per_layer = c->p.grid_num[1] * c->p.grid_num[2];
    for (int k = 0; k < n; ++k)
        if (layers[k] < 0 || layers[k] > c->p.grid_num[0]) return sph_fail(c, SPH_E_INVALID, "layer out of range");
    if (n > 8 && (size_t)n * 8 <= c->stage_bytes) {
        int* dl = (int*)c->stage;
        int* dout = dl + n;
        SPH_HIP(c, hipMemcpyAsync(dl, layers, (size_t)n * 4, hipMemcpyHostToDevice, c->stream));
        hipLaunchKernelGGL(k_read_layer_offsets, dim3((n + 255) / 256), dim3(256), 0, c->stream, c->cell_end, dl, n, per_layer, dout);
        SPH_LAUNCH_CHECK(c);
        SPH_HIP(c, hipMemcpyAsync(out, dout, (size_t)n * 4, hipMemcpyDeviceToHost, c->stream));
        SPH_HIP(c, hipStreamSynchronize(c->stream));
        return 0;
    }
    for (int k = 0; k < n; ++k) {
        const int L = layers[k];
        if (L == 0) out[k] = 0;
        else SPH_HIP(c, hipMemcpyAsync(&out[k], c->cell_end + (size_t)L * per_layer - 1, sizeof(int), hipMemcpyDeviceToHost, c->stream));
    }
    SPH_HIP(c, hipStreamSynchronize(c->stream));
    return 0;
}

static int layer_offset_cells(SphContext* c, const int32_t* layers, int32_t n, CellIdx16* ix) {
    const int per_layer = c->p.grid_num[1] * c->p.grid_num[2];
    c->off_zero_mask = 0;
    for (int k = 0; k < 16; ++k) ix->v[k] = -1;
    for (int k = 0; k < n; ++k) {
        const int L = layers[k];
        if (L < 0 || L > c->p.grid_num[0]) return sph_fail(c, SPH_E_INVALID, "layer out of range");
        if (L == 0) { c->off_zero_mask |= 1 << k; continue; }
        ix->v[k] = L * per_layer - 1;
    }
    return 0;
}

int32_t sph_layer_offsets_begin(SphContext* c, const int32_t* layers, int32_t n) {
    ENTER(c);
    c->off_stamp_pending = false;
    if (!layers || n < 0 || n > 16) return SPH_E_INVALID;
    if (!c->have_prefix) return sph_fail(c, SPH_E_STATE, "sph_layer_offsets_begin needs the prefix sum");
    CellIdx16 ix;
    int rc0 = layer_offset_cells(c, layers, n, &ix);
    if (rc0) return rc0;
    int* dev_out = nullptr;
    SPH_HIP(c, hipHostGetDevicePointer((void**)&dev_out, c->h_pinned, 0));
    hipLaunchKernelGGL(k_read_cells, dim3(1), dim3(64), 0, c->stream, c->cell_end, ix, dev_out);
    SPH_LAUNCH_CHECK(c);
    SPH_HIP(c, hipEventRecord(c->ev_off, c->stream));
    return 0;
}

int32_t sph_layer_offsets_end(SphContext* c, int32_t* out, int32_t n) {
    ENTER(c);
    if (!out || n < 0 || n > 16) return SPH_E_INVALID;
    if (c->off_stamp_pending) {
        c->off_stamp_pending = false;
        volatile int* hp = c->h_pinned;
        long spins = 0;
        while (__atomic_load_n(&hp[17], __ATOMIC_ACQUIRE) != c->off_stamp) {
            ++spins;
            if (spins > 4096) sched_yield();
            if ((spins & 0xffff) == 0) {
                const hipError_t q = hipStreamQuery(c->stream);
                if (q == hipSuccess && __atomic_load_n(&hp[17], __ATOMIC_ACQUIRE) != c->off_stamp)
                    return sph_fail(c, SPH_E_STATE, "sph_layer_offsets_end: the sort finished without delivering the layer offsets");
                if (q != hipSuccess && q != hipErrorNotReady) SPH_HIP(c, q);
            }
        }
    } else {
        SPH_HIP(c, hipEventSynchronize(c->ev_off));
    }
    for (int k = 0; k < n; ++k) out[k] = (c->off_zero_mask >> k) & 1 ? 0 : c->h_pinned[k];
    return 0;
}

int32_t sph_select_range(SphContext* c, int32_t first, int32_t count) {
    ENTER(c);
    if (first < 0 || count < 0 || first + count > c->in_off + c->N) return sph_fail(c, SPH_E_INVALID, "sph_select_range: out of range");
    c->in_off += first;
    c->N = count;
    sph_forget_pure_fluid(c);
    sphd_set_changed(c->dv);
    c->have_keys = c->have_prefix = c->sorted = false;
    c->n_dyn_host = -1;
    return 0;
}

int32_t sph_truncate(SphContext* c, int32_t n) {
    if (!c || n < 0 || n > c->N) return sph_fail(c, SPH_E_INVALID, "sph_truncate: out of range");
    if (n != c->N && !c->opt_no_dynamic) c->n_dyn_host = -1;
    if (n != c->N) sph_forget_pure_fluid(c);
    c->N = n;
    return 0;
}

int32_t sph_pack_range(SphContext* c, int32_t first, int32_t count, void* dst) {
    ENTER(c);
    if (first < 0 || count < 0 || first + count > c->N || (count > 0 && !dst)) return sph_fail(c, SPH_E_INVALID, "sph_pack_range: out of range");
    if (count == 0) return 0;
    const size_t b = (size_t)count * 16, o = (size_t)c->in_off + first;
    char* d = (char*)dst;
    SPH_HIP(c, hipMemcpyAsync(d, c->xm[c->cur] + o, b, hipMemcpyDeviceToDevice, c->stream));
    SPH_HIP(c, hipMemcpyAsync(d + b, c->vf[c->cur] + o, b, hipMemcpyDeviceToDevice, c->stream));
    SPH_HIP(c, hipMemcpyAsync(d + 2 * b, c->aux[c->cur] + o, b, hipMemcpyDeviceToDevice, c->stream));
    return 0;
}

int32_t sph_append_records(SphContext* c, const void* src, int32_t count) {
    ENTER(c);
    if (count < 0 || (count > 0 && !src)) return SPH_E_INVALID;
    if (c->in_off + c->N + count > c->cap) return sph_fail(c, SPH_E_NOMEM, "sph_append_records: capacity exceeded");
    if (count == 0) return 0;
    const size_t b = (size_t)count * 16, o = (size_t)c->in_off + c->N;
    const char* s = (const char*)src;
    SPH_HIP(c, hipMemcpyAsync(c->xm[c->cur] + o, s, b, hipMemcpyDeviceToDevice, c->stream));
    SPH_HIP(c, hipMemcpyAsync(c->vf[c->cur] + o, s + b, b, hipMemcpyDeviceToDevice, c->stream));
    SPH_HIP(c, hipMemcpyAsync(c->aux[c->cur] + o, s + 2 * b, b, hipMemcpyDeviceToDevice, c->stream));
    c->N += count;
    if (c->opt_uniform != 1) c->uniform_state = -1;
    sph_forget_pure_fluid(c);
    sph_invalidate_lists(c);
    c->have_keys = c->have_prefix = c->sorted = false;
    c->n_dyn_host = -1;
    return 0;
}

int32_t sph_sync(SphContext* c) {
    ENTER(c);
    SPH_HIP(c, hipStreamSynchronize(c->stream));
    return sph_check_device_flags(c);
}

int32_t sph_get_timings(SphContext* c, SphTimings* out) {
    ENTER(c);
    if (!out) return SPH_E_INVALID;
    int rc = harvest_events(c);
    rc = rc ? rc : sph_check_device_flags(c);
    if (rc) return rc;
    *out = c->tm;
    return 0;
}

int32_t sph_get_stats(SphContext* c, SphStats* out) {
    ENTER(c);
    if (!out) return SPH_E_INVALID;
    if (!c->have_prefix) return sph_fail(c, SPH_E_STATE, "sph_get_stats needs a sorted state (run a step first)");
    int rc = sphk_stats(c, out);
    return rc ? rc : sph_check_device_flags(c);
}

int32_t sph_reset_timings(SphContext* c) {
    ENTER(c);
    int rc = harvest_events(c);
    if (rc) return rc;
    memset(&c->tm, 0, sizeof(c->tm));
    return 0;
}

int32_t sph_slab_pack(SphContext* c, int32_t firstL, int32_t nL, void* dstL, int32_t firstR, int32_t nR, void* dstR) {
    ENTER(c);
    int rc = sph_pack_range(c, firstL, nL, dstL);
    rc = rc ? rc : sph_pack_range(c, firstR, nR, dstR);
    if (rc) return rc;
    SPH_HIP(c, hipStreamSynchronize(c->stream));
    return 0;
}

int32_t sph_slab_advance(SphContext* c, int32_t keep_first, int32_t keep_count, const void* srcL, int32_t nL,
                         const void* srcR, int32_t nR, const int32_t* layers, int32_t n_layers, int32_t do_sweeps) {
    ENTER(c);
    hipEvent_t* ev = nullptr;
    c->slab_ev_open = false;
    if (do_sweeps == 2) { int rt = timed_step_begin(c, &ev); if (rt) return rt; }
    int rc = do_sweeps == 0 ? sph_ensure_aux(c) : 0;
    rc = rc ? rc : sph_select_range(c, keep_first, keep_count);
    rc = rc ? rc : sph_append_records(c, srcL, nL);
    rc = rc ? rc : sph_append_records(c, srcR, nR);
    if (!rc && (!layers || n_layers < 0 || n_layers > 16)) rc = SPH_E_INVALID;
    CellIdx16 offset_cells;
    if (!rc) rc = layer_offset_cells(c, layers, n_layers, &offset_cells);
    if (!rc) c->off_stamp_pending = false;
    rc = rc ? rc : sort_no_fold(c, &offset_cells);
    if (!rc && !c->off_stamp_pending) c->off_zero_mask = 0xffff;
    if (!rc && ev) SPH_HIP(c, hipEventRecord(ev[1], c->stream));
    if (!rc && do_sweeps == 1) rc = sph_sweeps(c);
    if (!rc && do_sweeps == 2) {
        rc = refresh_dyn(c);
        rc = rc ? rc : density_phase(c);
        if (!rc && ev) { SPH_HIP(c, hipEventRecord(ev[2], c->stream)); c->slab_ev_open = true; }
    }
    return rc;
}

int32_t sph_slab_forces(SphContext* c, int32_t bl_lo, int32_t bl_hi, int32_t br_lo, int32_t br_hi,
                        int32_t firstL, int32_t nL, void* dstL, int32_t firstR, int32_t nR, void* dstR) {
    ENTER(c);
    int rc = need_sorted(c, "sph_slab_forces");
    if (rc) return rc;
    if (!c->opt_fused || c->opt_gather_impl != 1) return sph_fail(c, SPH_E_STATE, "sph_slab_forces needs the fused brick sweeps");
    if (firstL < 0 || nL < 0 || firstL + nL > c->N || firstR < 0 || nR < 0 || firstR + nR > c->N ||
        (nL > 0 && !dstL) || (nR > 0 && !dstR))
        return sph_fail(c, SPH_E_INVALID, "sph_slab_forces: bad pack range");
    const int f_lo = c->tgt_layers[2], f_hi = c->tgt_layers[3];
    bl_lo = bl_lo < f_lo ? f_lo : bl_lo; bl_hi = bl_hi > f_hi ? f_hi : bl_hi;
    br_hi = br_hi > f_hi ? f_hi : br_hi; br_lo = br_lo < bl_hi ? bl_hi : br_lo;
    if (bl_hi < bl_lo) bl_hi = bl_lo;
    if (br_lo > br_hi) br_lo = br_hi;
    static const bool no_side_env = getenv("SPH_NO_SIDE_STREAM") != nullptr;
    const bool no_boundary = bl_hi <= f_lo && br_lo >= f_hi && nL == 0 && nR == 0;
    const bool no_side = no_side_env || no_boundary;
    if (!no_side) {
        SPH_HIP(c, hipEventRecord(c->ev_fork, c->stream));
        SPH_HIP(c, hipStreamWaitEvent(c->side, c->ev_fork, 0));
    }
    SweepArgs boundary;
    boundary.lo = f_lo; boundary.hi = bl_hi; boundary.lo2 = br_lo; boundary.hi2 = f_hi;
    boundary.side = !no_side;
    const hipStream_t bst = no_side ? c->stream : c->side;
    rc = sphk_gather_layers(c, GM_FORCE_FUSED, boundary);
    rc = rc ? rc : sphk_fold_coupling_range(c, firstL, nL, bst);
    rc = rc ? rc : sphk_fold_coupling_range(c, firstR, nR, bst);
    rc = rc ? rc : sphk_pack_advected(c, firstL, nL, dstL, bst);
    rc = rc ? rc : sphk_pack_advected(c, firstR, nR, dstR, bst);
    if (rc) return rc;
    if (!no_boundary) SPH_HIP(c, hipEventRecord(c->ev_pack, bst));
    const bool fuse = c->uniform_state == 1 && sphd_one_gather_wcsph(c->dv) && c->opt_no_dynamic;
    SweepArgs interior;
    interior.lo = bl_hi; interior.hi = br_lo;
    interior.fuse_advect = fuse;
    interior.store_acc = !fuse;
    rc = sphk_gather_layers(c, GM_FORCE_FUSED, interior);
    c->acc_partial = fuse;
    if (rc) return rc;
    if (!no_boundary) SPH_HIP(c, hipStreamWaitEvent(c->stream, c->ev_pack, 0));
    hipEvent_t* ev = c->slab_ev_open ? c->ev[c->ev_used] : nullptr;
    if (ev) SPH_HIP(c, hipEventRecord(ev[3], c->stream));
    if (c->n_dyn_host != 0) { rc = sphk_fold_coupling(c); if (rc) return rc; }
    if (fuse) {
        const int a0 = firstL, a1 = firstL + nL, b0 = firstR, b1 = firstR + nR;
        if (nL > 0 && nR > 0 && b0 < a1) {
            const int lo = a0 < b0 ? a0 : b0, hi = a1 > b1 ? a1 : b1;
            rc = sphk_advect_range(c, lo, hi - lo);
        } else {
            rc = sphk_advect_range(c, firstL, nL);
            rc = rc ? rc : sphk_advect_range(c, firstR, nR);
        }
    } else {
        rc = sphk_advect(c, true);
    }
    if (!rc && ev) { SPH_HIP(c, hipEventRecord(ev[4], c->stream)); c->ev_used++; c->slab_ev_open = false; }
    return rc;
}

int32_t sph_slab_density(SphContext* c) {
    ENTER(c);
    int rc = need_sorted(c, "sph_slab_density");
    rc = rc ? rc : refresh_dyn(c);
    return rc ? rc : density_phase(c);
}

int32_t sph_rigid_partial_sums(SphContext* c, int32_t object_id, int32_t first, int32_t count, double* dev_sums16) {
    ENTER(c);
    if (object_id < 0 || object_id >= c->p.n_objects || !dev_sums16 || first < 0 || count < 0 || first + count > c->N)
        return sph_fail(c, SPH_E_INVALID, "sph_rigid_partial_sums: bad arguments");
    int rc = refresh_dyn(c);
    return rc ? rc : sphk_rigid_partial16(c, object_id, first, count, dev_sums16);
}

int32_t sph_rigid_apply_sums(SphContext* c, int32_t object_id, const double* dev_sums16, int32_t mode) {
    ENTER(c);
    if (object_id < 0 || object_id >= c->p.n_objects || !dev_sums16 || (mode != 0 && mode != 1))
        return sph_fail(c, SPH_E_INVALID, "sph_rigid_apply_sums: bad arguments");
    int rc = refresh_dyn(c);
    return rc ? rc : sphk_rigid_apply16(c, object_id, dev_sums16, mode);
}

int32_t sph_upload_rest_positions(SphContext* c, const int32_t* pid, const float* x0, int32_t n) {
    ENTER(c);
    if (n < 0 || (n > 0 && (!pid || !x0))) return sph_fail(c, SPH_E_INVALID, "sph_upload_rest_positions: bad arguments");
    const int chunk = (int)(c->stage_bytes / 16);
    for (int done = 0; done < n; done += chunk) {
        const int m = n - done < chunk ? n - done : chunk;
        int* dpid = (int*)c->stage;
        float* dx0 = (float*)((char*)c->stage + (size_t)m * 4);
        SPH_HIP(c, hipMemcpyAsync(dpid, pid + done, (size_t)m * 4, hipMemcpyHostToDevice, c->stream));
        SPH_HIP(c, hipMemcpyAsync(dx0, x0 + 3 * (size_t)done, (size_t)m * 12, hipMemcpyHostToDevice, c->stream));
        int rc = sphk_scatter_rest(c, dpid, dx0, m);
        if (rc) return rc;
        SPH_HIP(c, hipStreamSynchronize(c->stream));
    }
    return 0;
}

int32_t sph_dfsph_set_params(SphContext* c, const SphDfsphParams* p) {
    if (!c || !p) return SPH_E_INVALID;
    if (p->m_max_iterations_v < 0 || p->m_max_iterations < 0 || p->fluid_particle_num < 0)
        return sph_fail(c, SPH_E_INVALID, "sph_dfsph_set_params: negative count");
    c->df = *p;
    return 0;
}

int32_t sph_dfsph_get_stats(SphContext* c, SphDfsphStats* out) {
    if (!c || !out) return SPH_E_INVALID;
    *out = c->df_stats;
    return 0;
}

#define DF_SWEEP(NAME, MODE)                         \
    int32_t NAME(SphContext* c) {                    \
        ENTER(c);                                    \
        int rc = need_sorted(c, #NAME);              \
        rc = rc ? rc : refresh_dyn(c);               \
        return rc ? rc : sphk_gather(c, MODE);       \
    }
DF_SWEEP(sph_dfsph_compute_densities, GM_DF_DENSITY)
DF_SWEEP(sph_dfsph_compute_DFSPH_factor, GM_DF_FACTOR)
DF_SWEEP(sph_dfsph_compute_density_change, GM_DF_DENSITY_CHANGE)
DF_SWEEP(sph_dfsph_compute_density_adv, GM_DF_DENSITY_ADV)
DF_SWEEP(sph_dfsph_divergence_solver_iteration_kernel, GM_DF_DIV_ITER)
DF_SWEEP(sph_dfsph_pressure_solve_iteration_kernel, GM_DF_PRESSURE_ITER)
DF_SWEEP(sph_dfsph_compute_non_pressure_forces, GM_DF_NONPRESSURE)
#undef DF_SWEEP

int32_t sph_dfsph_compute_density_error(SphContext* c, float offset, float* out) {
    ENTER(c);
    if (!out) return SPH_E_INVALID;
    return sphk_df_density_error(c, offset, out);
}

int32_t sph_dfsph_compute_density_error_range(SphContext* c, float offset, int32_t first, int32_t count, double* out) {
    ENTER(c);
    if (!out || first < 0 || count < 0 || first + count > c->N) return sph_fail(c, SPH_E_INVALID, "sph_dfsph_compute_density_error_range: bad range");
    return sphk_df_density_error_range(c, offset, first, count, out);
}

int32_t sph_copy_velocity_records(SphContext* c, int32_t first, int32_t count, void* device_buf, int32_t to_context) {
    ENTER(c);
    if (first < 0 || count < 0 || first + count > c->N || (count > 0 && !device_buf))
        return sph_fail(c, SPH_E_INVALID, "sph_copy_velocity_records: bad range");
    if (count == 0) return 0;
    float4* vf = c->vf[c->cur] + (size_t)c->in_off + first;
    if (to_context) SPH_HIP(c, hipMemcpyAsync(vf, device_buf, (size_t)count * 16, hipMemcpyDeviceToDevice, c->stream));
    else SPH_HIP(c, hipMemcpyAsync(device_buf, vf, (size_t)count * 16, hipMemcpyDeviceToDevice, c->stream));
    return 0;
}

int32_t sph_dfsph_multiply_time_step(SphContext* c, float time_step) {
    ENTER(c);
    return sphk_df_scale_factor(c, time_step);
}

int32_t sph_dfsph_predict_velocity(SphContext* c) {
    ENTER(c);
    return sphk_df_predict_velocity(c);
}

int32_t sph_dfsph_advect(SphContext* c) {
    ENTER(c);
    return sphk_df_advect(c, false);
}

struct DfSolve { int sweep, refresh; float offset; double eta; int limit; };

static int df_enqueue_body(SphContext* c, const DfSolve& s, int k) {
    int rc = sphk_gather(c, s.sweep);
    SweepArgs refresh;
    refresh.collect_bpart = c->opt_df_fuse_err != 0;
    sphd_bpart_consumed(c->dv);
    rc = rc ? rc : sphk_gather(c, s.refresh, refresh);
    rc = rc ? rc : sphk_df_convergence_test(c, s.offset, s.eta, k & 3);
    if (rc) return rc;
    SPH_HIP(c, hipEventRecord(c->ev_df[k & 3], c->stream));
    return 0;
}

static int df_solve_loop(SphContext* c, const DfSolve& s, int* iterations, double* avg_err, int64_t* total) {
    c->df_epoch = c->df_epoch_done + 1u;
    if (c->df_epoch == 0u) {
        SPH_HIP(c, hipMemsetAsync(c->df_gate, 0, sizeof(unsigned), c->stream));
        c->df_epoch = 1u;
    }
    int rc = df_enqueue_body(c, s, 0);
    int k = 0;
    double avg = 0.0;
    while (!rc) {
        const bool more = k + 1 < s.limit;
        const bool ahead = more && c->opt_df_runahead;
        if (ahead) rc = df_enqueue_body(c, s, k + 1);
        if (rc) break;
        if (hipEventSynchronize(c->ev_df[k & 3]) != hipSuccess) { rc = sph_fail(c, SPH_E_STATE, "DFSPH solver: event wait failed"); break; }
        if ((rc = sph_check_device_flags(c)) != 0) break;
        const volatile SphContext::DfSlot* slot = c->h_df_slot + (k & 3);
        *total += 1;
        avg = slot->avg;
        if (slot->converged) break;
        k += 1;
        if (!more) break;
        if (!ahead) rc = df_enqueue_body(c, s, k);
    }
    c->df_epoch_done = c->df_epoch;
    c->df_epoch = 0u;
    *iterations = k;
    *avg_err = avg;
    return rc;
}

int32_t sph_dfsph_divergence_solve(SphContext* c) {
    ENTER(c);
    int rc = need_sorted(c, "sph_dfsph_divergence_solve");
    rc = rc ? rc : refresh_dyn(c);
    if (rc) return rc;
    const double dt = (double)c->p.dt;
    const double inv_dt = 1 / dt;
    rc = sphk_df_scale_factor(c, (float)inv_dt);
    rc = rc ? rc : sphk_gather(c, GM_DF_DENSITY_CHANGE);
    if (rc) return rc;
    DfSolve s;
    s.sweep = GM_DF_DIV_ITER; s.refresh = GM_DF_DENSITY_CHANGE; s.offset = 0.0f;
    s.eta = 1.0 / dt * c->df.max_error_V * 0.01 * (double)c->p.density_0;
    s.limit = c->df.m_max_iterations_v > 1 ? c->df.m_max_iterations_v : 1;
    int it = 0;
    double avg = 0.0;
    rc = df_solve_loop(c, s, &it, &avg, &c->df_stats.total_iterations_v);
    if (rc) return rc;
    c->df_stats.iterations_v = it;
    c->df_stats.avg_density_err_v = avg;
    return sphk_df_scale_factor(c, (float)dt);
}

int32_t sph_dfsph_pressure_solve(SphContext* c) {
    ENTER(c);
    int rc = need_sorted(c, "sph_dfsph_pressure_solve");
    rc = rc ? rc : refresh_dyn(c);
    if (rc) return rc;
    const double dt = (double)c->p.dt;
    const double inv_dt2 = 1 / (dt * dt);
    rc = sphk_df_scale_factor(c, (float)inv_dt2);
    rc = rc ? rc : sphk_gather(c, GM_DF_DENSITY_ADV);
    if (rc) return rc;
    DfSolve s;
    s.sweep = GM_DF_PRESSURE_ITER; s.refresh = GM_DF_DENSITY_ADV; s.offset = c->p.density_0;
    s.eta = c->df.max_error * 0.01 * (double)c->p.density_0;
    s.limit = c->df.m_max_iterations > 1 ? c->df.m_max_iterations : 1;
    int it = 0;
    double avg = 0.0;
    rc = df_solve_loop(c, s, &it, &avg, &c->df_stats.total_iterations);
    if (rc) return rc;
    c->df_stats.iterations = it;
    c->df_stats.avg_density_err = avg;
    return 0;
}

static int dfsph_sweeps(SphContext* c, hipEvent_t* ev, const int32_t* dynamic_ids, int32_t n_dynamic, bool) {
    int rc = c->n_dyn_host > 0 ? sphk_gather(c, GM_BVOL_DYNAMIC) : 0;
    rc = rc ? rc : sphk_gather(c, GM_DF_DENSITY);
    rc = rc ? rc : sphk_gather(c, GM_DF_FACTOR);
    if (rc) return rc;
    if (ev) SPH_HIP(c, hipEventRecord(ev[2], c->stream));
    if (c->df.enable_divergence_solver) { rc = sph_dfsph_divergence_solve(c); if (rc) return rc; }
    rc = sphk_gather(c, GM_DF_NONPRESSURE);
    rc = rc ? rc : sphk_df_predict_velocity(c);
    rc = rc ? rc : sph_dfsph_pressure_solve(c);
    if (rc) return rc;
    if (ev) SPH_HIP(c, hipEventRecord(ev[3], c->stream));
    rc = sphk_df_advect(c, true);
    if (rc) return rc;
    if (c->n_dyn_host > 0) { rc = sphk_rigid_solve_all(c, dynamic_ids, n_dynamic, false); if (rc) return rc; }
    c->df_stats.steps++;
    return 0;
}

int32_t sph_dfsph_step(SphContext* c, int32_t n_steps, const int32_t* dynamic_ids, int32_t n_dynamic) {
    ENTER(c);
    return step_loop(c, "sph_dfsph_step", dfsph_sweeps, n_steps, dynamic_ids, n_dynamic);
}

#ifdef SPH_PROFILE
int32_t sph_profile_read(SphContext* c, void* host, size_t bytes) {
    ENTER(c);
    if (!host || bytes > c->stage_bytes) return sph_fail(c, SPH_E_INVALID, "sph_profile_read: bad size");
    SPH_HIP(c, hipMemcpyAsync(host, c->stage, bytes, hipMemcpyDeviceToHost, c->stream));
    SPH_HIP(c, hipStreamSynchronize(c->stream));
    return 0;
}
#endif

static bool finite3(const double* v) { return isfinite(v[0]) && isfinite(v[1]) && isfinite(v[2]); }
static bool finite3f(const float* v) { return isfinite(v[0]) && isfinite(v[1]) && isfinite(v[2]); }

int32_t sph_kinematic_set(SphContext* c, const SphKinematicMotion* motions, int32_t n) {
    ENTER(c);
    if (sph_is_slab(c)) return sph_fail(c, SPH_E_STATE, "sph_kinematic_set: this context is a slab rank; kinematic bodies exist on single-domain contexts only");
    if (n < 0 || n > SPH_MAX_KINEMATIC || (n > 0 && !motions)) return sph_fail(c, SPH_E_INVALID, "sph_kinematic_set: n must be in [0, SPH_MAX_KINEMATIC] (and motions non-null)");
    for (int k = 0; k < n; ++k) {
        const SphKinematicMotion& m = motions[k];
        if (!finite3f(m.pivot) || !finite3(m.lin_vel) || !finite3(m.ang_vel) || !finite3(m.osc_amplitude) || !isfinite(m.osc_frequency) ||
            !isfinite(m.osc_phase) || !isfinite(m.start_time) || isnan(m.end_time) || m.end_time == -INFINITY) {
            snprintf(c->err, sizeof(c->err), "sph_kinematic_set: motion %d (object %d) has a non-finite field", k, m.object_id);
            return SPH_E_INVALID;
        }
        if (m.end_time < m.start_time) return sph_fail(c, SPH_E_INVALID, "sph_kinematic_set: end_time < start_time");
        for (int j = 0; j < k; ++j)
            if (motions[j].object_id == m.object_id) return sph_fail(c, SPH_E_INVALID, "sph_kinematic_set: an object id is given twice");
    }
    if (n > 0) {
        int rc = sph_obj_info(c);
        for (int k = 0; k < n && !rc; ++k) rc = kin_check_object(c, "sph_kinematic_set", motions[k].object_id);
        if (rc) return rc;
    }
    c->n_kin = n;
    for (int k = 0; k < n; ++k) c->kin[k] = motions[k];
    return 0;
}

int32_t sph_kinematic_apply(SphContext* c, const SphBodyPose* poses, int32_t n) {
    ENTER(c);
    if (sph_is_slab(c)) return sph_fail(c, SPH_E_STATE, "sph_kinematic_apply: this context is a slab rank; kinematic bodies exist on single-domain contexts only");
    if (n < 0 || n > SPH_MAX_KINEMATIC || (n > 0 && !poses)) return sph_fail(c, SPH_E_INVALID, "sph_kinematic_apply: n must be in [0, SPH_MAX_KINEMATIC] (and poses non-null)");
    if (n == 0) return 0;
    for (int k = 0; k < n; ++k) {
        const SphBodyPose& b = poses[k];
        bool fin = finite3f(b.pivot) && finite3f(b.origin) && finite3f(b.lin_vel) && finite3f(b.ang_vel);
        for (int j = 0; j < 9; ++j) fin = fin && isfinite(b.R[j]);
        if (!fin) {
            snprintf(c->err, sizeof(c->err), "sph_kinematic_apply: pose %d (object %d) has a non-finite field", k, b.object_id);
            return SPH_E_INVALID;
        }
        for (int i = 0; i < 3; ++i)
            for (int j = i; j < 3; ++j) {
                double dot = 0.0;
                for (int l = 0; l < 3; ++l) dot += (double)b.R[3 * i + l] * (double)b.R[3 * j + l];
                if (fabs(dot - (i == j ? 1.0 : 0.0)) > 1e-4) {
                    snprintf(c->err, sizeof(c->err), "sph_kinematic_apply: R of pose %d (object %d) is not orthonormal to 1e-4", k, b.object_id);
                    return SPH_E_INVALID;
                }
            }
        const double det = (double)b.R[0] * ((double)b.R[4] * b.R[8] - (double)b.R[5] * b.R[7]) - (double)b.R[1] * ((double)b.R[3] * b.R[8] - (double)b.R[5] * b.R[6]) +
                           (double)b.R[2] * ((double)b.R[3] * b.R[7] - (double)b.R[4] * b.R[6]);
        if (det < 0.0) {
            snprintf(c->err, sizeof(c->err), "sph_kinematic_apply: R of pose %d (object %d) is a reflection (det = -1)", k, b.object_id);
            return SPH_E_INVALID;
        }
        for (int j = 0; j < k; ++j)
            if (poses[j].object_id == b.object_id) return sph_fail(c, SPH_E_INVALID, "sph_kinematic_apply: an object id is given twice");
    }
    int rc = sph_obj_info(c);
    if (rc) return rc;
    KinPoses P;
    P.n = n;
    for (int k = 0; k < SPH_MAX_KINEMATIC; ++k) P.id[k] = -1;
    for (int k = 0; k < n; ++k) {
        const SphBodyPose& b = poses[k];
        rc = kin_check_object(c, "sph_kinematic_apply", b.object_id);
        if (rc) return rc;
        double R[9], pivot[3], origin[3];
        for (int j = 0; j < 9; ++j) R[j] = (double)b.R[j];
        for (int a = 0; a < 3; ++a) { pivot[a] = (double)b.pivot[a]; origin[a] = (double)b.origin[a]; }
        if (!kin_contained(c, b.object_id, R, pivot, origin)) {
            snprintf(c->err, sizeof(c->err), "sph_kinematic_apply: object %d would leave [padding, domain - padding]; nothing was enqueued", b.object_id);
            return SPH_E_INVALID;
        }
        P.id[k] = b.object_id;
        memcpy(P.R[k], b.R, sizeof(b.R));
        memcpy(P.pivot[k], b.pivot, sizeof(b.pivot));
        memcpy(P.origin[k], b.origin, sizeof(b.origin));
        memcpy(P.lin[k], b.lin_vel, sizeof(b.lin_vel));
        memcpy(P.ang[k], b.ang_vel, sizeof(b.ang_vel));
    }
    return sphk_kinematic_apply(c, P);
}

int32_t sph_get_time(SphContext* c, double* t) {
    if (!c || !t) return SPH_E_INVALID;
    *t = c->sim_time;
    return 0;
}

int32_t sph_set_time(SphContext* c, double t) {
    if (!c) return SPH_E_INVALID;
    if (!isfinite(t)) return sph_fail(c, SPH_E_INVALID, "sph_set_time: the time must be finite");
    c->sim_time = t;
    return 0;
}

int32_t sph_slab_wait_pack(SphContext* c) {
    ENTER(c);
    SPH_HIP(c, hipEventSynchronize(c->ev_pack));
    return 0;
}

}
```

### sph_taichi_amd/csrc/sph_derived.h

```cpp
#pragma once

struct SphPartKey {
    int id;
    int lo, hi, lo2, hi2;
    bool operator==(const SphPartKey& o) const { return id == o.id && lo == o.lo && hi == o.hi && lo2 == o.lo2 && hi2 == o.hi2; }
    bool inside(const SphPartKey& o) const {
        const bool in1 = lo >= o.lo && hi <= o.hi;
        const bool in2 = lo2 == hi2 || (lo2 >= o.lo && hi2 <= o.hi);
        return id == o.id && o.lo2 == o.hi2 && in1 && in2;
    }
};

enum SphPartHit { SPH_PART_NO = 0, SPH_PART_SUBSET = 1, SPH_PART_EXACT = 2 };

struct SphDerived {
    bool lists_valid;
    bool gcnt_written;
    int stg_kind;
    int k_kind;
    bool bricks_valid;
    SphPartKey bricks_key;
    bool brec_valid;
    SphPartKey brec_key;
    bool df_bpart_valid;
    bool aux_stale;
    bool brick_count_zero;
};

static inline void sphd_invalidate(SphDerived& s) { s.lists_valid = s.bricks_valid = s.brec_valid = false; s.stg_kind = s.k_kind = 0; }
static inline void sphd_set_changed(SphDerived& s) { sphd_invalidate(s); s.aux_stale = false; }
static inline void sphd_sorted(SphDerived& s, bool built, const SphPartKey& key) {
    sphd_set_changed(s);
    s.gcnt_written = false;
    s.brick_count_zero = false;
    s.bricks_valid = built;
    if (built) s.bricks_key = key;
}
static inline void sphd_partition_rebuilt(SphDerived& s, const SphPartKey& key) {
    s.lists_valid = s.brec_valid = false;
    s.brick_count_zero = false;
    s.bricks_valid = true;
    s.bricks_key = key;
}
static inline void sphd_lists_written(SphDerived& s, int stg_kind) {
    s.lists_valid = s.gcnt_written = true;
    s.stg_kind = stg_kind;
    s.k_kind = 0;
    if (stg_kind == 1) s.aux_stale = true;
}
static inline void sphd_records_written(SphDerived& s, const SphPartKey& key) { s.brec_valid = true; s.brec_key = key; }
static inline void sphd_k_written(SphDerived& s, int kind) { s.k_kind = kind; }
static inline void sphd_bpart_written(SphDerived& s) { s.df_bpart_valid = true; }
static inline void sphd_bpart_consumed(SphDerived& s) { s.df_bpart_valid = false; }
static inline void sphd_aux_folded(SphDerived& s) { s.aux_stale = false; }
static inline void sphd_count_zeroed(SphDerived& s, bool zero) { s.brick_count_zero = zero; }

static inline SphPartHit sphd_partition_hit(const SphDerived& s, const SphPartKey& key) {
    if (!s.bricks_valid) return SPH_PART_NO;
    return key == s.bricks_key ? SPH_PART_EXACT : key.inside(s.bricks_key) ? SPH_PART_SUBSET : SPH_PART_NO;
}
static inline bool sphd_lists_usable(const SphDerived& s) { return s.lists_valid; }
static inline bool sphd_records_usable(const SphDerived& s, const SphPartKey& key) { return s.lists_valid && s.brec_valid && key == s.brec_key; }
static inline bool sphd_one_gather_wcsph(const SphDerived& s) { return s.lists_valid && s.stg_kind == 1; }
static inline bool sphd_one_gather_df(const SphDerived& s, int k_kind) { return s.lists_valid && s.stg_kind == 2 && s.k_kind == k_kind; }
static inline bool sphd_stats_have_lists(const SphDerived& s) { return s.gcnt_written; }
static inline bool sphd_bpart_ready(const SphDerived& s) { return s.df_bpart_valid; }
static inline bool sphd_aux_in_eos2(const SphDerived& s) { return s.aux_stale; }
static inline bool sphd_count_is_zero(const SphDerived& s) { return s.brick_count_zero; }
```

### sph_taichi_amd/csrc/sph_internal.h

```cpp
#pragma once
#include <hip/hip_runtime.h>
#include <stdint.h>
#include <stdio.h>
#include <string.h>

#include "../../include/sph_hip.h"
#include "sph_derived.h"

#define SPH_MATERIAL_SOLID 0
#define SPH_MATERIAL_FLUID 1
#define SPH_MAX_TIMED_STEPS 128
#define SPH_GLIST_ROWS 96
#define SPH_DF_ERR_BLOCKS 512
#define SPH_VAR_PURE_INTERNAL 64
#define SPH_VAR_DEFAULT (SPH_VAR_GROUPS | SPH_VAR_FORCE_BF | SPH_VAR_DEEP)

struct DevView {
    int N, G;
    int nx, ny, nz;
    int ox, oy, oz;
    int tgt_lo, tgt_hi;
    int tgt_lo2, tgt_hi2;
    int sort_by_pid;
    int drop_outside;
    int exp_int;
    double* df_bpart;
    const unsigned* gate;
    unsigned gate_epoch;
#ifdef SPH_PROFILE
    int ablate;
    unsigned long long* prof_ts;
#endif
    float grid_size, h, inv_h, d2, m_V0, rho0, stiffness, exponent, sigma, dt;
    float gx, gy, gz;
    float pad;
    float k_w, k_dw, visc_d_nu, visc_eps;
    float w_zero, w_d;
    float m_eps;
    float m_u;
    double fx_scale;
    float whx, why, whz;
    int fuse_advect;
    int write_sg;
    int write_k;
    int store_acc;
    int rigid_from_x0;
    float4* xm;
    float4* vf;
    float4* aux;
    float4* eos;
    float2* eos2;
    float4* stg;
    float4* gat;
    float* kbuf;
    float4* acc;
    long long* acc_fx;
    int* key;
    int* cell_end;
    const float* x0_cold;
    int* polar_fb;
    float* rigid_rest_cm;
};

struct SphRender;
struct SphDiag;
struct SphColumns;
struct SphExport;
struct SphSurface;
struct CellIdx16 { int v[16]; };

struct SphContext {
    SphParams p;
    int device;
    hipStream_t stream;
    bool own_stream;
    int N;
    int cap;
    int cold_cap;
    int G;
    int cur;
    int* h_pinned;
    hipEvent_t ev_off;
    hipEvent_t ev_pack;
    hipEvent_t ev_fork;
    hipStream_t side;
    int2* brick_list2;
    int* brick_count2;
    int off_zero_mask;
    int off_stamp;
    bool off_stamp_pending;
    int tgt_layers[4];
    int nx_alloc;
    int in_off;
    float4* xm[2];
    float4* vf[2];
    float4* aux[2];
    int* key[2];
    float4* eos;
    float2* eos2;
    float4* stg;
    float4* gat;
    float4* acc;
    float4* acc_tmp;
    long long* acc_fx;
    int* cell_end;
    int* cell_buf[2];
    int cell_cur;
    bool next_cells_zero;
    int* rank_off;
    int* idx_unstable;
    unsigned long long* scan_status;
    unsigned scan_epoch;
    int* scan_err;
    unsigned short* glist;
    int glist_shift;
    unsigned char* gcnt;
    int4* brick_rec;
    int opt_brick_rec;
    int2* brick_list;
    int* brick_count;
    int brick_cap;
    int scan_blocks;
    float* x0_cold;
    int* color_cold;
    float* rigid_rest_cm;
    int* dyn_list;
    int* dyn_count;
    int n_dyn_host;
    int rigid_fx_exp;
    double* rigid_part;
    int rigid_part_blocks;
    float* rigid_R;
    void* stage;
    size_t stage_bytes;
    bool have_keys, have_prefix, sorted;
    SphDerived dv;
    double* h_df_err;
    struct DfSlot { float err; int converged; double avg; }* h_df_slot;
    unsigned* df_gate;
    unsigned df_epoch;
    unsigned df_epoch_done;
    hipEvent_t ev_df[4];
    double* df_part;
    double* df_bpart;
    int opt_df_fuse_err;
    SphDfsphParams df;
    SphDfsphStats df_stats;
    double* df_err;
    int timing_phase;
    int opt_gather_impl, opt_timing, opt_fused, opt_brick_shape, opt_no_dynamic, opt_ablate, opt_drop_outside;
    int opt_sort_by_pid;
    int opt_rigid_batch;
    int opt_df_runahead;
    int opt_exact_math;
    int opt_rigid_x0;
    int opt_pure_instance;
    int opt_variant;
    bool acc_partial;
    int opt_uniform;
    int uniform_state;
    int pure_fluid;
    int pure_fluid_n;
    float m_uniform;
    hipEvent_t ev[SPH_MAX_TIMED_STEPS][5];
    int ev_used;
    bool slab_ev_open;
    SphTimings tm;
    SphRender* render;
    SphDiag* diag;
    SphColumns* columns;
    SphExport* exporter;
    SphSurface* surface;
    double sim_time;
    int n_kin;
    SphKinematicMotion kin[SPH_MAX_KINEMATIC];
    struct ObjInfo { int n, n_static; double lo[3], hi[3]; }* obj_info;
    bool obj_info_valid;
    char err[512];
};

DevView sph_view(const SphContext* c);
#define SPH_BRICK_HEAVY 160
static inline void sph_invalidate_lists(SphContext* c) { sphd_invalidate(c->dv); }
int sph_fail(SphContext* c, int code, const char* what);
static inline bool sph_is_slab(const SphContext* c) {
    return c->p.cell_origin[0] != 0 || c->p.cell_origin[1] != 0 || c->p.cell_origin[2] != 0 || c->p.cold_capacity > 0 ||
           c->p.grid_num[0] != c->nx_alloc || c->opt_drop_outside || c->in_off != 0;
}
static inline void sph_forget_pure_fluid(SphContext* c) { c->pure_fluid = 0; c->pure_fluid_n = -1; }
static inline bool sph_pure_fluid_instances(const SphContext* c) {
    const bool pure_checked = c->opt_pure_instance == 1 && c->pure_fluid && c->pure_fluid_n == c->N && !c->opt_drop_outside;
    return c->uniform_state == 1 && (pure_checked || c->opt_pure_instance == 2);
}
int sph_check_device_flags(SphContext* c);

#define SPH_HIP(ctx, expr)                                                        \
    do {                                                                          \
        hipError_t e__ = (expr);                                                  \
        if (e__ != hipSuccess) {                                                  \
            snprintf((ctx)->err, sizeof((ctx)->err), "%s: %s (%s:%d)", #expr,     \
                     hipGetErrorString(e__), __FILE__, __LINE__);                 \
            return (int)e__;                                                      \
        }                                                                         \
    } while (0)

#define SPH_LAUNCH_CHECK(ctx) SPH_HIP(ctx, hipGetLastError())

int sphk_hash_histogram(SphContext* c);
int sphk_scan(SphContext* c);
int sphk_sort_scatter(SphContext* c, bool sort_acc, const CellIdx16* deliver_offsets);
int sphk_rigid_partial16(SphContext* c, int object_id, int first, int count, double* out);
int sphk_rigid_apply16(SphContext* c, int object_id, const double* sums, int mode);
int sphk_scatter_rest(SphContext* c, const int* pid_dev, const float* x0_dev, int n);
struct BrickListArgs;
int sphk_brick_list_prepare(SphContext* c, BrickListArgs* a, SphPartKey* key);
struct SweepArgs {
    int lo = -1, hi = -1, lo2 = 0, hi2 = 0;
    bool fuse_advect = false;
    bool store_acc = true;
    bool collect_bpart = false;
    bool side = false;
};
int sphk_gather(SphContext* c, int mode, const SweepArgs& a = SweepArgs());
int sphk_gather_layers(SphContext* c, int mode, const SweepArgs& a);
int sphk_pack_advected(SphContext* c, int first, int count, void* dst, hipStream_t st);
int sphk_eos(SphContext* c);
int sph_ensure_aux(SphContext* c);
int sphk_stats(SphContext* c, SphStats* out);
int sphk_df_convergence_test(SphContext* c, float offset, double eta, int slot);
int sphk_check_uniform_fluid(SphContext* c);
int sphk_df_density_error(SphContext* c, float offset, float* out_host);
int sphk_df_density_error_range(SphContext* c, float offset, int first, int count, double* out_host);
int sphk_df_scale_factor(SphContext* c, float s);
int sphk_df_predict_velocity(SphContext* c);
int sphk_df_advect(SphContext* c, bool fused_fluid_walls);
int sphk_advect(SphContext* c, bool fused_fluid_walls);
int sphk_advect_dyn_list(SphContext* c);
int sphk_fold_coupling_range(SphContext* c, int first, int count, hipStream_t st);
int sphk_fold_coupling(SphContext* c);
int sphk_advect_range(SphContext* c, int first, int count);
int sphk_enforce_boundary(SphContext* c, int particle_type);
int sphk_rigid_com(SphContext* c, int object_id, bool to_rest);
int sphk_rigid_solve(SphContext* c, int object_id);
int sphk_rigid_solve_all(SphContext* c, const int* ids, int n_ids, bool advect_first);
int sphk_extract(SphContext* c, int field, void* dst);
struct KinPoses { int n; int id[SPH_MAX_KINEMATIC]; float R[SPH_MAX_KINEMATIC][9], pivot[SPH_MAX_KINEMATIC][3], origin[SPH_MAX_KINEMATIC][3], lin[SPH_MAX_KINEMATIC][3], ang[SPH_MAX_KINEMATIC][3]; };
int sphk_rest_records(SphContext* c, float4* dst);
int sphk_kinematic_apply(SphContext* c, const KinPoses& poses);
int sphk_insert(SphContext* c, int field, const void* src);
void sph_render_release(SphContext* c);
void sph_diag_release(SphContext* c);
void sph_columns_release(SphContext* c);
void sph_export_release(SphContext* c);
void sph_surface_release(SphContext* c);

enum GatherMode {
    GM_BVOL_STATIC = 0,
    GM_BVOL_DYNAMIC = 1,
    GM_DENSITY = 2,
    GM_DENSITY_EOS = 3,
    GM_NONPRESSURE = 4,
    GM_PRESSURE = 5,
    GM_FORCE_FUSED = 6,
    GM_DF_DENSITY = 7,
    GM_DF_FACTOR = 8,
    GM_DF_DENSITY_CHANGE = 9,
    GM_DF_DENSITY_ADV = 10,
    GM_DF_DIV_ITER = 11,
    GM_DF_PRESSURE_ITER = 12,
    GM_DF_NONPRESSURE = 13,
    GM_FORCE_FUSED_U = 14,
    GM_DF_DIV_ITER_U = 15,
    GM_DF_PRESSURE_ITER_U = 16
};

#ifdef __HIPCC__
__device__ __forceinline__ int sph_flags_material(int f) { return f & 0xFF; }
__device__ __forceinline__ int sph_flags_dynamic(int f) { return (f >> 8) & 1; }
__device__ __forceinline__ int sph_flags_object(int f) { return (int)((unsigned)f >> 9); }
__device__ __forceinline__ bool sph_is_fluid(int f) { return (f & 0xFF) == SPH_MATERIAL_FLUID; }
__device__ __forceinline__ bool sph_is_static_rigid(int f) { return (f & 0x1FF) == 0; }
__device__ __forceinline__ bool sph_is_dynamic_rigid(int f) { return (f & 0x1FF) == 0x100; }

__device__ __forceinline__ int sph_cell_coord(float p, float grid_size, int origin, int n) {
    int c = (int)(p / grid_size) - origin;
    c = c < 0 ? 0 : c;
    c = c > n - 1 ? n - 1 : c;
    return c;
}
__device__ __forceinline__ int sph_flatten(const DevView& d, int cx, int cy, int cz) {
    return (cx * d.ny + cy) * d.nz + cz;
}

__device__ __forceinline__ int sph_wave_inclusive_scan(int v, int lane) {
#pragma unroll
    for (int off = 1; off < 64; off <<= 1) {
        int n = __shfl_up(v, off, 64);
        if (lane >= off) v += n;
    }
    return v;
}

template <bool FAST>
__device__ __forceinline__ float sph_tait_pow(const DevView& d, float x) {
    if (d.exp_int > 0) {
        float r = 1.0f, b = x;
        for (int e = d.exp_int; e; e >>= 1) {
            if (e & 1) r *= b;
            b *= b;
        }
        return r;
    }
    return FAST ? __builtin_amdgcn_exp2f(d.exponent * __builtin_amdgcn_logf(x)) : powf(x, d.exponent);
}

__device__ __forceinline__ void wall_collide(const DevView& d, const float hi[3], float4& xm, float4& vf) {
    const float pos[3] = {xm.x, xm.y, xm.z};
    float x[3] = {xm.x, xm.y, xm.z};
    float n[3] = {0.f, 0.f, 0.f};
#pragma unroll
    for (int a = 0; a < 3; ++a) {
        if (pos[a] > hi[a]) { n[a] += 1.0f; x[a] = hi[a]; }
        if (pos[a] <= d.pad) { n[a] += -1.0f; x[a] = d.pad; }
    }
    xm.x = x[0]; xm.y = x[1]; xm.z = x[2];
    const float len = sqrtf(n[0] * n[0] + n[1] * n[1] + n[2] * n[2]);
    if (len > 1e-6f) {
        const float vx_ = n[0] / len, vy_ = n[1] / len, vz_ = n[2] / len;
        const float vd = vf.x * vx_ + vf.y * vy_ + vf.z * vz_;
        vf.x -= (1.0f + 0.5f) * vd * vx_;
        vf.y -= (1.0f + 0.5f) * vd * vy_;
        vf.z -= (1.0f + 0.5f) * vd * vz_;
    }
}


template <bool FLUID_WALLS>
__device__ __forceinline__ void advect_one(const DevView& d, const float hi[3], float4& xm, float4& vf, const float4 a) {
    const int fl = __float_as_int(vf.w);
    if (!sph_flags_dynamic(fl)) return;
    vf.x += d.dt * a.x; vf.y += d.dt * a.y; vf.z += d.dt * a.z;
    xm.x += d.dt * vf.x; xm.y += d.dt * vf.y; xm.z += d.dt * vf.z;
    if (FLUID_WALLS && sph_is_fluid(fl)) wall_collide(d, hi, xm, vf);
}


#endif
```

### sph_taichi_amd/csrc/sph_sort.hip

```cpp
#include "sph_internal.h"
#include "sph_bricks.h"

#define TPB 256
#define SCAN_IPT 8
#define SCAN_TILE (TPB * SCAN_IPT)

__global__ __launch_bounds__(TPB) void k_hash_histogram(DevView d, int* __restrict__ cell_cnt,
                                                        int* __restrict__ rank_off, int* __restrict__ brick_count) {
    const int i = blockIdx.x * TPB + threadIdx.x;
    const int lane = threadIdx.x & 63;
    if (i == 0) brick_count[0] = brick_count[1] = 0;
    int c = -1 - lane;
    if (i < d.N) {
        const float4 p = d.xm[i];
        const int cx = sph_cell_coord(p.x, d.grid_size, d.ox, d.nx);
        const int cy = sph_cell_coord(p.y, d.grid_size, d.oy, d.ny);
        const int cz = sph_cell_coord(p.z, d.grid_size, d.oz, d.nz);
        c = sph_flatten(d, cx, cy, cz);
        if (d.drop_outside) {
            const int raw = (int)(p.x / d.grid_size) - d.ox;
            if (raw < 0 || raw >= d.nx) c = d.G;
        }
        d.key[i] = c;
    }
    const int prev = __shfl_up(c, 1, 64);
    const bool head = (lane == 0) || (prev != c);
    const unsigned long long heads = __ballot(head);
    const unsigned long long below = heads & (~0ull >> (63 - lane));
    const int head_lane = 63 - __clzll(below);
    const unsigned long long above = (head_lane == 63) ? 0ull : (heads >> (head_lane + 1));
    const int run_len = above ? (__ffsll((long long)above)) : (64 - head_lane);
    int base = 0;
    if (head && c >= 0) base = atomicAdd(&cell_cnt[c], run_len);
    base = __shfl(base, head_lane, 64);
    if (i < d.N) rank_off[i] = base + (lane - head_lane);
}

__device__ __forceinline__ int block_exclusive_offset(int thread_total, int* s_wave, int& block_total) {
    const int lane = threadIdx.x & 63, wave = threadIdx.x >> 6;
    const int incl = sph_wave_inclusive_scan(thread_total, lane);
    if (lane == 63) s_wave[wave] = incl;
    __syncthreads();
    int wave_off = 0, tot = 0;
#pragma unroll
    for (int w = 0; w < TPB / 64; ++w) {
        const int s = s_wave[w];
        if (w < wave) wave_off += s;
        tot += s;
    }
    block_total = tot;
    return wave_off + incl - thread_total;
}

#define SCAN_SPIN_LIMIT (1 << 22)
__global__ __launch_bounds__(TPB) void k_scan_fused(int4* __restrict__ data, unsigned long long* __restrict__ status,
                                                    unsigned epoch, int* __restrict__ err) {
    __shared__ int s_wave[TPB / 64];
    const int base = (blockIdx.x * TPB + threadIdx.x) * (SCAN_IPT / 4);
    int4 v[SCAN_IPT / 4];
    int t = 0;
#pragma unroll
    for (int k = 0; k < SCAN_IPT / 4; ++k) {
        v[k] = data[base + k];
        t += v[k].x + v[k].y + v[k].z + v[k].w;
    }
    int tot;
    const int ex = block_exclusive_offset(t, s_wave, tot);
    if (threadIdx.x == 0)
        __hip_atomic_store(&status[blockIdx.x], ((unsigned long long)epoch << 32) | (unsigned)tot, __ATOMIC_RELAXED,
                           __HIP_MEMORY_SCOPE_AGENT);
    int before = 0;
    for (int j = threadIdx.x; j < (int)blockIdx.x; j += TPB) {
        unsigned long long w;
        int spins = 0;
        do {
            w = __hip_atomic_load(&status[j], __ATOMIC_RELAXED, __HIP_MEMORY_SCOPE_AGENT);
        } while ((unsigned)(w >> 32) != epoch && ++spins < SCAN_SPIN_LIMIT);
        if ((unsigned)(w >> 32) != epoch) { *err = 1; w = 0ull; }
        before += (int)(unsigned)w;
    }
    __syncthreads();
    int before_tot;
    (void)block_exclusive_offset(before, s_wave, before_tot);
    int run = before_tot + ex;
#pragma unroll
    for (int k = 0; k < SCAN_IPT / 4; ++k) {
        run += v[k].x; v[k].x = run;
        run += v[k].y; v[k].y = run;
        run += v[k].z; v[k].z = run;
        run += v[k].w; v[k].w = run;
        data[base + k] = v[k];
    }
}

__global__ __launch_bounds__(TPB) void k_unstable_place(DevView d, const int* __restrict__ rank_off,
                                                        int* __restrict__ idx_unstable, int* __restrict__ dyn_count,
                                                        CellIdx16 off_ix, int* __restrict__ off_out, int off_stamp) {
    const int i = blockIdx.x * TPB + threadIdx.x;
    if (i == 0) *dyn_count = 0;
    if (off_out != nullptr && i == 0) {
        int v[16];
#pragma unroll
        for (int k = 0; k < 16; ++k) v[k] = off_ix.v[k] >= 0 ? d.cell_end[off_ix.v[k]] : 0;
#pragma unroll
        for (int k = 0; k < 16; ++k) __hip_atomic_store(&off_out[k], v[k], __ATOMIC_RELAXED, __HIP_MEMORY_SCOPE_SYSTEM);
        __atomic_thread_fence(__ATOMIC_RELEASE);
        __hip_atomic_store(&off_out[17], off_stamp, __ATOMIC_RELEASE, __HIP_MEMORY_SCOPE_SYSTEM);
    }
    if (i >= d.N) return;
    const int c = d.key[i];
    const int b = c > 0 ? d.cell_end[c - 1] : 0;
    idx_unstable[b + rank_off[i]] = i;
}

template <bool SORT_ACC>
__global__ __launch_bounds__(TPB) void k_stable_scatter(DevView d, const int* __restrict__ idx_unstable,
                                                        float4* __restrict__ xm_out, float4* __restrict__ vf_out,
                                                        float4* __restrict__ aux_out, int* __restrict__ key_out,
                                                        float4* __restrict__ acc_out, int* __restrict__ dyn_list,
                                                        int* __restrict__ dyn_count, int4* __restrict__ zero_dst,
                                                        int zero_n4, BrickListArgs bl) {
    extern __shared__ int sm_bl[];
    if ((int)blockIdx.x < bl.nblocks) {
        sph_brick_list_block<SPH_BRICK_BX, SPH_BRICK_BY, SPH_BRICK_BZ>(bl.d, bl.nbx, bl.nby, bl.list, bl.count, bl.list_cap, bl.tmax,
                                                                        bl.smax, bl.fixed_bz, (int)blockIdx.x, sm_bl);
        return;
    }
    const int s = ((int)blockIdx.x - bl.nblocks) * TPB + threadIdx.x;
    for (int z = s; z < zero_n4; z += ((int)gridDim.x - bl.nblocks) * TPB) zero_dst[z] = make_int4(0, 0, 0, 0);
    const bool live = s < d.N;
    const int lane = threadIdx.x & 63;
    const int i = live ? idx_unstable[s] : 0;
    const int c = live ? d.key[i] : 0;
    const int b = c > 0 ? d.cell_end[c - 1] : 0;
    const int e = live ? d.cell_end[c] : 0;
    const int my = live ? (d.sort_by_pid ? __float_as_int(d.aux[i].w) : i) : 0;
    int rank = s - b;
    const bool ranked = live && c != d.G;
    const bool crowded = ranked && e - b > 64;
    if (ranked && !crowded) {
        rank = 0;
        if (d.sort_by_pid) {
            for (int t = b; t < e; ++t) rank += (__float_as_int(d.aux[idx_unstable[t]].w) < my) ? 1 : 0;
        } else {
            for (int t = b; t < e; ++t) rank += (idx_unstable[t] < my) ? 1 : 0;
        }
    }
    unsigned long long todo = __ballot(crowded);
    while (todo) {
        const int src = __ffsll((long long)todo) - 1;
        todo &= todo - 1ull;
        const int bb = __shfl(b, src, 64), ee = __shfl(e, src, 64), kk = __shfl(my, src, 64);
        int cnt = 0;
        for (int t = bb + lane; t < ee; t += 64) {
            const int v = idx_unstable[t];
            cnt += ((d.sort_by_pid ? __float_as_int(d.aux[v].w) : v) < kk) ? 1 : 0;
        }
#pragma unroll
        for (int off = 32; off > 0; off >>= 1) cnt += __shfl_xor(cnt, off, 64);
        if (lane == src) rank = cnt;
    }
    if (!live) return;
    const int dst = b + rank;
    const float4 xm = d.xm[i];
    const float4 vf = d.vf[i];
    const float4 aux = d.aux[i];
    xm_out[dst] = xm;
    vf_out[dst] = vf;
    aux_out[dst] = aux;
    key_out[dst] = c;
    if (SORT_ACC) acc_out[dst] = d.acc[i];
    if (c != d.G && sph_is_dynamic_rigid(__float_as_int(vf.w))) dyn_list[atomicAdd(dyn_count, 1)] = dst;
}

int sphk_hash_histogram(SphContext* c) {
    const int Gpad = c->scan_blocks * SCAN_TILE;
    int* nxt = c->cell_buf[c->cell_cur ^ 1];
    if (!c->next_cells_zero) SPH_HIP(c, hipMemsetAsync(nxt, 0, sizeof(int) * (size_t)Gpad, c->stream));
    c->cell_cur ^= 1;
    c->cell_end = nxt;
    c->next_cells_zero = false;
    sphd_count_zeroed(c->dv, c->N > 0);
    if (c->N > 0) {
        DevView d = sph_view(c);
        hipLaunchKernelGGL(k_hash_histogram, dim3((c->N + TPB - 1) / TPB), dim3(TPB), 0, c->stream, d, c->cell_end,
                           c->rank_off, c->brick_count);
        SPH_LAUNCH_CHECK(c);
    }
    return 0;
}

int sphk_scan(SphContext* c) {
    const int nb = c->scan_blocks;
    c->scan_epoch += 1u;
    if (c->scan_epoch == 0u) {
        SPH_HIP(c, hipMemsetAsync(c->scan_status, 0, (size_t)(nb + 1) * 8, c->stream));
        c->scan_epoch = 1u;
    }
    hipLaunchKernelGGL(k_scan_fused, dim3(nb), dim3(TPB), 0, c->stream, (int4*)c->cell_end, c->scan_status, c->scan_epoch,
                       c->scan_err);
    SPH_LAUNCH_CHECK(c);
    return 0;
}

int sphk_sort_scatter(SphContext* c, bool sort_acc, const CellIdx16* deliver_offsets) {
    if (c->N <= 0) return 0;
    DevView d = sph_view(c);
    const int nb = (c->N + TPB - 1) / TPB;
    const int o = c->cur ^ 1;
    int4* zero_dst = reinterpret_cast<int4*>(c->cell_buf[c->cell_cur ^ 1]);
    const int zero_n4 = c->scan_blocks * SCAN_TILE / 4;
    BrickListArgs bl;
    SphPartKey bl_key;
    int rc = sphk_brick_list_prepare(c, &bl, &bl_key);
    if (rc) return rc;
    if (bl.nblocks > 0 && !sphd_count_is_zero(c->dv)) {
        SPH_HIP(c, hipMemsetAsync(c->brick_count, 0, 2 * sizeof(int), c->stream));
    }
    CellIdx16 off_ix;
    int* off_out = nullptr;
    for (int k = 0; k < 16; ++k) off_ix.v[k] = -1;
    if (deliver_offsets) {
        off_ix = *deliver_offsets;
        SPH_HIP(c, hipHostGetDevicePointer((void**)&off_out, c->h_pinned, 0));
        c->off_stamp = c->off_stamp == 0x7fffffff ? 1 : c->off_stamp + 1;
        c->off_stamp_pending = true;
    }
    hipLaunchKernelGGL(k_unstable_place, dim3(nb), dim3(TPB), 0, c->stream, d, c->rank_off, c->idx_unstable, c->dyn_count, off_ix, off_out,
                       c->off_stamp);
    SPH_LAUNCH_CHECK(c);
    if (sort_acc)
        hipLaunchKernelGGL(k_stable_scatter<true>, dim3(nb + bl.nblocks), dim3(TPB), bl.lds_bytes, c->stream, d, c->idx_unstable, c->xm[o],
                           c->vf[o], c->aux[o], c->key[o], c->acc_tmp, c->dyn_list, c->dyn_count, zero_dst, zero_n4, bl);
    else
        hipLaunchKernelGGL(k_stable_scatter<false>, dim3(nb + bl.nblocks), dim3(TPB), bl.lds_bytes, c->stream, d, c->idx_unstable, c->xm[o],
                           c->vf[o], c->aux[o], c->key[o], c->acc_tmp, c->dyn_list, c->dyn_count, zero_dst, zero_n4, bl);
    SPH_LAUNCH_CHECK(c);
    c->next_cells_zero = true;
    c->cur = o;
    sphd_sorted(c->dv, bl.nblocks > 0, bl_key);
    if (sort_acc) {
        float4* t = c->acc;
        c->acc = c->acc_tmp;
        c->acc_tmp = t;
    }
    return 0;
}
```

Before: 2231.

## Add incremental fast sort that only relocates particles whose cell changed

Adds a fast sort path used during stepping when the previous order came from a sort. The hash kernel records only particles that changed cell, as per-cell deltas plus linked lists of arrivals. The scan adds those deltas to the previous cell_end, and a new scatter computes each particle's destination from the old offsets, the arrival lists and popcounts of movers, which avoids the full histogram atomics and the unstable place pass. It adds a third cell buffer, two head buffers, linked-list walks per particle and a bounds check that flags errors, with extra cost if many particles move or cells become crowded with arrivals.

Result: faster. 2298, median of 6 (+3.0%).

```diff
diff --git a/include/sph_hip.h b/include/sph_hip.h
--- a/include/sph_hip.h
+++ b/include/sph_hip.h
@@ -87,7 +87,10 @@
     SPH_OPT_RIGID_SUMS_FROM_X0 = 14,
     SPH_OPT_PURE_FLUID_INSTANCE = 15 ,
     SPH_OPT_BRICK_RECORDS = 16 ,
-    SPH_OPT_DF_FUSE_ERROR = 17
+    SPH_OPT_DF_FUSE_ERROR = 17 ,
+    SPH_OPT_SORT_FAST = 18     ,
+    SPH_OPT_SORT_FAST_COUNT = 19,
+    SPH_OPT_SORT_GENERAL_COUNT = 20
 };
 #define SPH_VAR_GROUPS 1
 #define SPH_VAR_MFMA 32
diff --git a/sph_taichi_amd/_lib.py b/sph_taichi_amd/_lib.py
--- a/sph_taichi_amd/_lib.py
+++ b/sph_taichi_amd/_lib.py
@@ -125,7 +125,8 @@
     F_IS_DYNAMIC, F_GRID_IDS, F_GRID_PARTICLES_NUM, F_PID, F_RIGID_REST_CM, F_DFSPH_FACTOR, F_DENSITY_ADV = range(18)
 OPT_GATHER_IMPL, OPT_TIMING, OPT_FUSED_STEP, OPT_BRICK_SHAPE, OPT_NO_DYNAMIC_SOLIDS, OPT_DEBUG_ABLATE, \
     OPT_SLAB_DROP_OUTSIDE, OPT_UNIFORM_FLUID, OPT_UNIFORM_FLUID_STATE, OPT_SORT_BY_PID, OPT_KERNEL_VARIANT, \
-    OPT_RIGID_BATCH, OPT_EXACT_MATH, OPT_DF_RUNAHEAD, OPT_RIGID_SUMS_FROM_X0, OPT_PURE_FLUID_INSTANCE, OPT_BRICK_RECORDS, OPT_DF_FUSE_ERROR = range(18)
+    OPT_RIGID_BATCH, OPT_EXACT_MATH, OPT_DF_RUNAHEAD, OPT_RIGID_SUMS_FROM_X0, OPT_PURE_FLUID_INSTANCE, OPT_BRICK_RECORDS, OPT_DF_FUSE_ERROR, \
+    OPT_SORT_FAST, OPT_SORT_FAST_COUNT, OPT_SORT_GENERAL_COUNT = range(21)
 VAR_GROUPS, VAR_GAT_LDS, VAR_GAT_LDS4, VAR_FORCE_BF, VAR_DEEP, VAR_MFMA = 1, 2, 4, 8, 16, 32
 VAR_DEFAULT = VAR_GROUPS | VAR_FORCE_BF | VAR_DEEP
 
diff --git a/sph_taichi_amd/csrc/sph_api.hip b/sph_taichi_amd/csrc/sph_api.hip
--- a/sph_taichi_amd/csrc/sph_api.hip
+++ b/sph_taichi_amd/csrc/sph_api.hip
@@ -79,7 +79,8 @@
         ((volatile int*)c->h_pinned)[16] = 0;
         c->sorted = c->have_prefix = c->have_keys = false;
         sph_invalidate_lists(c);
-        return sph_fail(c, SPH_E_STATE, "prefix sum: a scan tile never saw a predecessor's total (k_scan_fused's bounded wait ran out); "
+        sphd_records_moved(c->dv);
+        return sph_fail(c, SPH_E_STATE, "sort: a scan tile never saw a predecessor's total (k_scan_fused's bounded wait ran out), or a fast sort met a rank outside the arrays; "
                                         "the cell table of that sort and every result since are invalid: re-upload the state and sort again");
     }
     return 0;
@@ -286,6 +287,7 @@
     c->opt_brick_shape = 0;
     c->opt_rigid_batch = 1;
     c->opt_df_fuse_err = 1;
+    c->opt_sort_fast = SPH_SORT_FAST_DEFAULT;
     c->opt_df_runahead = 0;
     c->opt_exact_math = 0;
     c->opt_rigid_x0 = 0;
@@ -316,7 +318,11 @@
     rc = rc ? rc : alloc_dev(c, (void**)&c->acc_fx, cap * 3 * sizeof(long long));
     rc = rc ? rc : alloc_dev(c, (void**)&c->cell_buf[0], (size_t)c->scan_blocks * SCAN_TILE * 4);
     rc = rc ? rc : alloc_dev(c, (void**)&c->cell_buf[1], (size_t)c->scan_blocks * SCAN_TILE * 4);
-    if (!rc) { c->cell_cur = 0; c->cell_end = c->cell_buf[0]; c->next_cells_zero = false; }
+    rc = rc ? rc : alloc_dev(c, (void**)&c->cell_buf[2], (size_t)c->scan_blocks * SCAN_TILE * 4);
+    rc = rc ? rc : alloc_dev(c, (void**)&c->head_buf[0], (size_t)c->scan_blocks * SCAN_TILE * 4);
+    rc = rc ? rc : alloc_dev(c, (void**)&c->head_buf[1], (size_t)c->scan_blocks * SCAN_TILE * 4);
+    if (!rc) { c->cell_cur = 0; c->cell_prev = 2; c->cell_next = 1; c->cell_end = c->cell_buf[0]; c->next_cells_zero = false; }
+    if (!rc) { c->head_cur = 0; c->next_heads_zero = true; c->sort_fast_pending = false; c->n_sort_fast = c->n_sort_general = 0; }
     rc = rc ? rc : alloc_dev(c, (void**)&c->rank_off, cap * 4);
     rc = rc ? rc : alloc_dev(c, (void**)&c->idx_unstable, cap * 4);
     rc = rc ? rc : alloc_dev(c, (void**)&c->scan_status, (size_t)(c->scan_blocks + 1) * 8);
@@ -395,7 +401,7 @@
     (void)hipSetDevice(c->device);
     if (c->stream) (void)hipStreamSynchronize(c->stream);
     void* ptrs[] = {c->xm[0], c->xm[1], c->vf[0], c->vf[1], c->aux[0], c->aux[1], c->key[0], c->key[1], c->eos, c->stg, c->gat, c->acc,
-                    c->acc_tmp, c->cell_buf[0], c->cell_buf[1], c->rank_off, c->idx_unstable, c->scan_status, c->x0_cold, c->color_cold,
+                    c->acc_tmp, c->cell_buf[0], c->cell_buf[1], c->cell_buf[2], c->head_buf[0], c->head_buf[1], c->rank_off, c->idx_unstable, c->scan_status, c->x0_cold, c->color_cold,
                     c->rigid_rest_cm, c->dyn_list, c->dyn_count, c->acc_fx, c->rigid_part, c->rigid_R, c->df_err, c->df_part, c->df_bpart, c->stage, c->glist, c->gcnt, c->brick_list, c->brick_count, c->brick_list2, c->brick_count2, c->brick_rec};
     for (void* p : ptrs) if (p) (void)hipFree(p);
     sph_render_release(c);
@@ -451,6 +457,7 @@
             c->opt_pure_instance = value; sph_invalidate_lists(c); return 0;
         case SPH_OPT_BRICK_RECORDS: c->opt_brick_rec = value ? 1 : 0; sph_invalidate_lists(c); return 0;
         case SPH_OPT_DF_FUSE_ERROR: c->opt_df_fuse_err = value ? 1 : 0; return 0;
+        case SPH_OPT_SORT_FAST: c->opt_sort_fast = value ? 1 : 0; return 0;
     }
     return sph_fail(c, SPH_E_INVALID, "unknown option");
 }
@@ -476,6 +483,9 @@
         case SPH_OPT_PURE_FLUID_INSTANCE: *value = c->opt_pure_instance; return 0;
         case SPH_OPT_BRICK_RECORDS: *value = c->opt_brick_rec; return 0;
         case SPH_OPT_DF_FUSE_ERROR: *value = c->opt_df_fuse_err; return 0;
+        case SPH_OPT_SORT_FAST: *value = c->opt_sort_fast; return 0;
+        case SPH_OPT_SORT_FAST_COUNT: *value = c->n_sort_fast; return 0;
+        case SPH_OPT_SORT_GENERAL_COUNT: *value = c->n_sort_general; return 0;
     }
     return SPH_E_INVALID;
 }
@@ -535,6 +545,7 @@
     SPH_HIP(c, hipMemcpyAsync(c->stage, host, bytes, hipMemcpyHostToDevice, c->stream));
     int rc = sphk_insert(c, field, c->stage);
     if (rc) return rc;
+    sphd_records_moved(c->dv);
     SPH_HIP(c, hipStreamSynchronize(c->stream));
     if (field == SPH_F_MATERIAL || field == SPH_F_IS_DYNAMIC || field == SPH_F_DENSITY) c->n_dyn_host = -1;
     if (field == SPH_F_MATERIAL || field == SPH_F_M || field == SPH_F_M_V) c->uniform_state = -1;
@@ -593,15 +604,19 @@
     if (!(c)) return SPH_E_INVALID;               \
     SPH_HIP((c), hipSetDevice((c)->device));
 
-int32_t sph_update_grid_id(SphContext* c) {
-    ENTER(c);
-    int rc = sphk_hash_histogram(c);
+static int update_grid_id(SphContext* c, bool allow_fast) {
+    int rc = sphk_hash_histogram(c, allow_fast);
     if (rc) return rc;
     c->have_keys = true;
     c->have_prefix = false;
     return 0;
 }
 
+int32_t sph_update_grid_id(SphContext* c) {
+    ENTER(c);
+    return update_grid_id(c, false);
+}
+
 int32_t sph_prefix_sum(SphContext* c) {
     ENTER(c);
     if (!c->have_keys) return sph_fail(c, SPH_E_STATE, "sph_prefix_sum before sph_update_grid_id");
@@ -613,8 +628,10 @@
 
 static int counting_sort(SphContext* c, bool sort_acc, const CellIdx16* deliver_offsets = nullptr) {
     if (!c->have_prefix) return sph_fail(c, SPH_E_STATE, "sph_counting_sort before sph_prefix_sum");
+    const bool recount = c->n_dyn_host < 0;
     int rc = refresh_dyn(c);
     if (rc) return rc;
+    if (recount && c->sort_fast_pending) SPH_HIP(c, hipMemsetAsync(c->dyn_count, 0, sizeof(int), c->stream));
     rc = sphk_sort_scatter(c, sort_acc, deliver_offsets);
     if (rc) return rc;
     c->in_off = 0;
@@ -803,8 +820,8 @@
     return 0;
 }
 
-static int sort_no_fold(SphContext* c, const CellIdx16* deliver_offsets = nullptr) {
-    int rc = sph_update_grid_id(c);
+static int sort_no_fold(SphContext* c, const CellIdx16* deliver_offsets = nullptr, bool allow_fast = false) {
+    int rc = update_grid_id(c, allow_fast && !deliver_offsets);
     rc = rc ? rc : sph_prefix_sum(c);
     return rc ? rc : counting_sort(c, false, deliver_offsets);
 }
@@ -827,7 +844,9 @@
     c->tgt_layers[0] = c->tgt_layers[2] = 0;
     c->tgt_layers[1] = c->tgt_layers[3] = nx;
     c->next_cells_zero = false;
+    c->next_heads_zero = false;
     sph_invalidate_lists(c);
+    sphd_records_moved(c->dv);
     c->have_keys = c->have_prefix = c->sorted = false;
     c->n_dyn_host = -1;
     return 0;
@@ -866,7 +885,7 @@
         const double t_end = c->sim_time + (double)c->p.dt;
         hipEvent_t* ev = nullptr;
         rc = timed_step_begin(c, &ev);
-        rc = rc ? rc : sort_no_fold(c);
+        rc = rc ? rc : sort_no_fold(c, nullptr, true);
         if (rc) return rc;
         if (ev) SPH_HIP(c, hipEventRecord(ev[1], c->stream));
         rc = body(c, ev, dynamic_ids, n_dynamic, it + 1 == n_steps);
@@ -989,6 +1008,7 @@
     if (!c || n < 0 || n > c->N) return sph_fail(c, SPH_E_INVALID, "sph_truncate: out of range");
     if (n != c->N && !c->opt_no_dynamic) c->n_dyn_host = -1;
     if (n != c->N) sph_forget_pure_fluid(c);
+    sphd_records_moved(c->dv);
     c->N = n;
     return 0;
 }
@@ -1019,6 +1039,7 @@
     if (c->opt_uniform != 1) c->uniform_state = -1;
     sph_forget_pure_fluid(c);
     sph_invalidate_lists(c);
+    sphd_records_moved(c->dv);
     c->have_keys = c->have_prefix = c->sorted = false;
     c->n_dyn_host = -1;
     return 0;
diff --git a/sph_taichi_amd/csrc/sph_derived.h b/sph_taichi_amd/csrc/sph_derived.h
--- a/sph_taichi_amd/csrc/sph_derived.h
+++ b/sph_taichi_amd/csrc/sph_derived.h
@@ -25,10 +25,12 @@
     bool df_bpart_valid;
     bool aux_stale;
     bool brick_count_zero;
+    bool order_from_sort;
 };
 
 static inline void sphd_invalidate(SphDerived& s) { s.lists_valid = s.bricks_valid = s.brec_valid = false; s.stg_kind = s.k_kind = 0; }
-static inline void sphd_set_changed(SphDerived& s) { sphd_invalidate(s); s.aux_stale = false; }
+static inline void sphd_set_changed(SphDerived& s) { sphd_invalidate(s); s.aux_stale = false; s.order_from_sort = false; }
+static inline void sphd_records_moved(SphDerived& s) { s.order_from_sort = false; }
 static inline void sphd_sorted(SphDerived& s, bool built, const SphPartKey& key) {
     sphd_set_changed(s);
     s.gcnt_written = false;
@@ -36,6 +38,8 @@
     s.bricks_valid = built;
     if (built) s.bricks_key = key;
 }
+static inline void sphd_hash_started(SphDerived& s) { s.order_from_sort = false; }
+static inline void sphd_order_established(SphDerived& s, bool strays_possible) { s.order_from_sort = !strays_possible; }
 static inline void sphd_partition_rebuilt(SphDerived& s, const SphPartKey& key) {
     s.lists_valid = s.brec_valid = false;
     s.brick_count_zero = false;
@@ -67,3 +71,6 @@
 static inline bool sphd_bpart_ready(const SphDerived& s) { return s.df_bpart_valid; }
 static inline bool sphd_aux_in_eos2(const SphDerived& s) { return s.aux_stale; }
 static inline bool sphd_count_is_zero(const SphDerived& s) { return s.brick_count_zero; }
+static inline bool sphd_sort_fast_usable(const SphDerived& s, bool opt_fast, bool sort_by_pid, bool drop_outside) {
+    return opt_fast && s.order_from_sort && !sort_by_pid && !drop_outside;
+}
diff --git a/sph_taichi_amd/csrc/sph_internal.h b/sph_taichi_amd/csrc/sph_internal.h
--- a/sph_taichi_amd/csrc/sph_internal.h
+++ b/sph_taichi_amd/csrc/sph_internal.h
@@ -12,6 +12,7 @@
 #define SPH_MAX_TIMED_STEPS 128
 #define SPH_GLIST_ROWS 96
 #define SPH_DF_ERR_BLOCKS 512
+#define SPH_SORT_FAST_DEFAULT 1
 #define SPH_VAR_PURE_INTERNAL 64
 #define SPH_VAR_DEFAULT (SPH_VAR_GROUPS | SPH_VAR_FORCE_BF | SPH_VAR_DEEP)
 
@@ -104,9 +105,17 @@
     float4* acc_tmp;
     long long* acc_fx;
     int* cell_end;
-    int* cell_buf[2];
+    int* cell_buf[3];
     int cell_cur;
+    int cell_prev;
+    int cell_next;
     bool next_cells_zero;
+    int* head_buf[2];
+    int head_cur;
+    bool next_heads_zero;
+    bool sort_fast_pending;
+    int opt_sort_fast;
+    int n_sort_fast, n_sort_general;
     int* rank_off;
     int* idx_unstable;
     unsigned long long* scan_status;
@@ -206,7 +215,7 @@
 
 #define SPH_LAUNCH_CHECK(ctx) SPH_HIP(ctx, hipGetLastError())
 
-int sphk_hash_histogram(SphContext* c);
+int sphk_hash_histogram(SphContext* c, bool allow_fast = false);
 int sphk_scan(SphContext* c);
 int sphk_sort_scatter(SphContext* c, bool sort_acc, const CellIdx16* deliver_offsets);
 int sphk_rigid_partial16(SphContext* c, int object_id, int first, int count, double* out);
diff --git a/sph_taichi_amd/csrc/sph_sort.hip b/sph_taichi_amd/csrc/sph_sort.hip
--- a/sph_taichi_amd/csrc/sph_sort.hip
+++ b/sph_taichi_amd/csrc/sph_sort.hip
@@ -36,6 +36,29 @@
     if (i < d.N) rank_off[i] = base + (lane - head_lane);
 }
 
+__global__ __launch_bounds__(TPB) void k_hash_fast(DevView d, int* __restrict__ key_new, int* __restrict__ delta,
+                                                   int* __restrict__ head, int* __restrict__ next,
+                                                   int* __restrict__ brick_count, int* __restrict__ dyn_count) {
+    const int i = blockIdx.x * TPB + threadIdx.x;
+    if (i == 0) {
+        brick_count[0] = brick_count[1] = 0;
+        *dyn_count = 0;
+    }
+    if (i >= d.N) return;
+    const float4 p = d.xm[i];
+    const int cx = sph_cell_coord(p.x, d.grid_size, d.ox, d.nx);
+    const int cy = sph_cell_coord(p.y, d.grid_size, d.oy, d.ny);
+    const int cz = sph_cell_coord(p.z, d.grid_size, d.oz, d.nz);
+    const int c = sph_flatten(d, cx, cy, cz);
+    const int co = d.key[i];
+    key_new[i] = c;
+    if (c != co) {
+        atomicAdd(&delta[co], -1);
+        atomicAdd(&delta[c], 1);
+        next[i] = atomicExch(&head[c], i + 1);
+    }
+}
+
 __device__ __forceinline__ int block_exclusive_offset(int thread_total, int* s_wave, int& block_total) {
     const int lane = threadIdx.x & 63, wave = threadIdx.x >> 6;
     const int incl = sph_wave_inclusive_scan(thread_total, lane);
@@ -53,15 +76,26 @@
 }
 
 #define SCAN_SPIN_LIMIT (1 << 22)
+template <bool DELTA>
 __global__ __launch_bounds__(TPB) void k_scan_fused(int4* __restrict__ data, unsigned long long* __restrict__ status,
-                                                    unsigned epoch, int* __restrict__ err) {
+                                                    unsigned epoch, int* __restrict__ err, const int* __restrict__ old_end) {
     __shared__ int s_wave[TPB / 64];
     const int base = (blockIdx.x * TPB + threadIdx.x) * (SCAN_IPT / 4);
     int4 v[SCAN_IPT / 4];
     int t = 0;
+    int left = 0;
+    if (DELTA && base > 0) left = old_end[base * 4 - 1];
 #pragma unroll
     for (int k = 0; k < SCAN_IPT / 4; ++k) {
         v[k] = data[base + k];
+        if (DELTA) {
+            const int4 o = reinterpret_cast<const int4*>(old_end)[base + k];
+            v[k].x += o.x - left;
+            v[k].y += o.y - o.x;
+            v[k].z += o.z - o.y;
+            v[k].w += o.w - o.z;
+            left = o.w;
+        }
         t += v[k].x + v[k].y + v[k].z + v[k].w;
     }
     int tot;
@@ -173,14 +207,122 @@
     if (c != d.G && sph_is_dynamic_rigid(__float_as_int(vf.w))) dyn_list[atomicAdd(dyn_count, 1)] = dst;
 }
 
-int sphk_hash_histogram(SphContext* c) {
+__device__ __forceinline__ int sph_popc_range(unsigned long long w, int a, int b) {
+    if (a >= b) return 0;
+    const unsigned long long upto_b = b >= 64 ? ~0ull : ((1ull << b) - 1ull);
+    return __popcll(w & upto_b & ~((1ull << a) - 1ull));
+}
+
+template <bool SORT_ACC>
+__global__ __launch_bounds__(TPB) void k_stable_scatter_fast(DevView d, const int* __restrict__ old_end, const int* __restrict__ key_new,
+                                                             const int* __restrict__ head, const int* __restrict__ next,
+                                                             float4* __restrict__ xm_out, float4* __restrict__ vf_out,
+                                                             float4* __restrict__ aux_out, int* __restrict__ key_out,
+                                                             float4* __restrict__ acc_out, int* __restrict__ dyn_list,
+                                                             int* __restrict__ dyn_count, int4* __restrict__ zero_dst,
+                                                             int4* __restrict__ zero_head, int zero_n4, int* __restrict__ err,
+                                                             BrickListArgs bl) {
+    extern __shared__ int sm_bl[];
+    __shared__ unsigned long long s_mov[TPB / 64];
+    if ((int)blockIdx.x < bl.nblocks) {
+        sph_brick_list_block<SPH_BRICK_BX, SPH_BRICK_BY, SPH_BRICK_BZ>(bl.d, bl.nbx, bl.nby, bl.list, bl.count, bl.list_cap, bl.tmax,
+                                                                        bl.smax, bl.fixed_bz, (int)blockIdx.x, sm_bl);
+        return;
+    }
+    const int bs = ((int)blockIdx.x - bl.nblocks) * TPB;
+    const int s = bs + threadIdx.x;
+    for (int z = s; z < zero_n4; z += ((int)gridDim.x - bl.nblocks) * TPB) {
+        zero_dst[z] = make_int4(0, 0, 0, 0);
+        zero_head[z] = make_int4(0, 0, 0, 0);
+    }
+    const bool live = s < d.N;
+    const int lane = threadIdx.x & 63, wave = threadIdx.x >> 6;
+    const int co = live ? d.key[s] : 0;
+    const int c = live ? key_new[s] : 0;
+    const bool mover = live && c != co;
+    const unsigned long long movers = __ballot(mover);
+    if (lane == 0) s_mov[wave] = movers;
+    const int ob = (live && c > 0) ? old_end[c - 1] : 0;
+    const int nb = (live && c > 0) ? d.cell_end[c - 1] : 0;
+    int arrivals = 0, smaller = 0;
+    for (int a = live ? head[c] : 0; a != 0 && arrivals < d.N; a = next[a - 1]) {
+        ++arrivals;
+        smaller += (a - 1 < s) ? 1 : 0;
+    }
+    __syncthreads();
+    const bool stayer = live && !mover;
+    int gone = 0;
+    if (stayer) {
+        const int lo = (ob > bs ? ob : bs) - bs;
+#pragma unroll
+        for (int w = 0; w < TPB / 64; ++w) {
+            int a = lo - 64 * w, b = (int)threadIdx.x - 64 * w;
+            a = a < 0 ? 0 : a;
+            b = b > 64 ? 64 : b;
+            gone += sph_popc_range(s_mov[w], a, b);
+        }
+    }
+    const bool before = stayer && ob < bs;
+    const bool far = before && bs - ob > 64;
+    if (before && !far)
+        for (int j = ob; j < bs; ++j) gone += (d.key[j] != key_new[j]) ? 1 : 0;
+    unsigned long long todo = __ballot(far);
+    while (todo) {
+        const int src = __ffsll((long long)todo) - 1;
+        const int bb = __shfl(ob, src, 64);
+        int cnt = 0;
+        for (int j = bb + lane; j < bs; j += 64) cnt += (d.key[j] != key_new[j]) ? 1 : 0;
+#pragma unroll
+        for (int off = 32; off > 0; off >>= 1) cnt += __shfl_xor(cnt, off, 64);
+        const bool mine = far && ob == bb;
+        if (mine) gone += cnt;
+        todo &= ~__ballot(mine);
+    }
+    if (!live) return;
+    int dst;
+    if (mover) {
+        const int stayers = d.cell_end[c] - nb - arrivals;
+        dst = nb + smaller + (s >= ob ? stayers : 0);
+    } else {
+        dst = nb + smaller + (s - ob) - gone;
+    }
+    if ((unsigned)dst >= (unsigned)d.N) { *err = 1; return; }
+    const float4 xm = d.xm[s];
+    const float4 vf = d.vf[s];
+    const float4 aux = d.aux[s];
+    xm_out[dst] = xm;
+    vf_out[dst] = vf;
+    aux_out[dst] = aux;
+    key_out[dst] = c;
+    if (SORT_ACC) acc_out[dst] = d.acc[s];
+    if (sph_is_dynamic_rigid(__float_as_int(vf.w))) dyn_list[atomicAdd(dyn_count, 1)] = dst;
+}
+
+int sphk_hash_histogram(SphContext* c, bool allow_fast) {
     const int Gpad = c->scan_blocks * SCAN_TILE;
-    int* nxt = c->cell_buf[c->cell_cur ^ 1];
+    const bool fast = allow_fast && c->N > 0 && c->in_off == 0 &&
+                      sphd_sort_fast_usable(c->dv, c->opt_sort_fast != 0, c->opt_sort_by_pid != 0, c->opt_drop_outside != 0);
+    sphd_hash_started(c->dv);
+    int* nxt = c->cell_buf[c->cell_next];
     if (!c->next_cells_zero) SPH_HIP(c, hipMemsetAsync(nxt, 0, sizeof(int) * (size_t)Gpad, c->stream));
-    c->cell_cur ^= 1;
+    const int old_cur = c->cell_cur;
+    c->cell_cur = c->cell_next;
+    c->cell_prev = old_cur;
+    c->cell_next = 3 - c->cell_cur - c->cell_prev;
     c->cell_end = nxt;
     c->next_cells_zero = false;
     sphd_count_zeroed(c->dv, c->N > 0);
+    c->sort_fast_pending = fast;
+    if (fast) {
+        if (!c->next_heads_zero) SPH_HIP(c, hipMemsetAsync(c->head_buf[c->head_cur ^ 1], 0, sizeof(int) * (size_t)Gpad, c->stream));
+        c->head_cur ^= 1;
+        c->next_heads_zero = false;
+        DevView d = sph_view(c);
+        hipLaunchKernelGGL(k_hash_fast, dim3((c->N + TPB - 1) / TPB), dim3(TPB), 0, c->stream, d, c->rank_off, c->cell_end,
+                           c->head_buf[c->head_cur], c->idx_unstable, c->brick_count, c->dyn_count);
+        SPH_LAUNCH_CHECK(c);
+        return 0;
+    }
     if (c->N > 0) {
         DevView d = sph_view(c);
         hipLaunchKernelGGL(k_hash_histogram, dim3((c->N + TPB - 1) / TPB), dim3(TPB), 0, c->stream, d, c->cell_end,
@@ -197,9 +339,28 @@
         SPH_HIP(c, hipMemsetAsync(c->scan_status, 0, (size_t)(nb + 1) * 8, c->stream));
         c->scan_epoch = 1u;
     }
-    hipLaunchKernelGGL(k_scan_fused, dim3(nb), dim3(TPB), 0, c->stream, (int4*)c->cell_end, c->scan_status, c->scan_epoch,
-                       c->scan_err);
+    if (c->sort_fast_pending)
+        hipLaunchKernelGGL(k_scan_fused<true>, dim3(nb), dim3(TPB), 0, c->stream, (int4*)c->cell_end, c->scan_status, c->scan_epoch,
+                           c->scan_err, c->cell_buf[c->cell_prev]);
+    else
+        hipLaunchKernelGGL(k_scan_fused<false>, dim3(nb), dim3(TPB), 0, c->stream, (int4*)c->cell_end, c->scan_status, c->scan_epoch,
+                           c->scan_err, (const int*)nullptr);
     SPH_LAUNCH_CHECK(c);
+    return 0;
+}
+
+static int sort_scatter_done(SphContext* c, int o, int zeroed, bool sort_acc, bool built, const SphPartKey& key) {
+    c->cell_next = zeroed;
+    c->next_cells_zero = true;
+    c->cur = o;
+    const bool strays_possible = c->opt_drop_outside != 0;
+    sphd_sorted(c->dv, built, key);
+    sphd_order_established(c->dv, strays_possible);
+    if (sort_acc) {
+        float4* t = c->acc;
+        c->acc = c->acc_tmp;
+        c->acc_tmp = t;
+    }
     return 0;
 }
 
@@ -208,7 +369,10 @@
     DevView d = sph_view(c);
     const int nb = (c->N + TPB - 1) / TPB;
     const int o = c->cur ^ 1;
-    int4* zero_dst = reinterpret_cast<int4*>(c->cell_buf[c->cell_cur ^ 1]);
+    const bool fast = c->sort_fast_pending && !deliver_offsets;
+    if (c->sort_fast_pending && !fast) return sph_fail(c, SPH_E_STATE, "sort: layer offsets cannot ride in a fast sort");
+    const int zero_ix = fast ? 3 - c->cell_cur - c->cell_prev : c->cell_prev;
+    int4* zero_dst = reinterpret_cast<int4*>(c->cell_buf[zero_ix]);
     const int zero_n4 = c->scan_blocks * SCAN_TILE / 4;
     BrickListArgs bl;
     SphPartKey bl_key;
@@ -216,6 +380,24 @@
     if (rc) return rc;
     if (bl.nblocks > 0 && !sphd_count_is_zero(c->dv)) {
         SPH_HIP(c, hipMemsetAsync(c->brick_count, 0, 2 * sizeof(int), c->stream));
+    }
+    if (fast) {
+        const int* old_end = c->cell_buf[c->cell_prev];
+        const int* head = c->head_buf[c->head_cur];
+        int4* zero_head = reinterpret_cast<int4*>(c->head_buf[c->head_cur ^ 1]);
+        if (sort_acc)
+            hipLaunchKernelGGL(k_stable_scatter_fast<true>, dim3(nb + bl.nblocks), dim3(TPB), bl.lds_bytes, c->stream, d, old_end, c->rank_off,
+                               head, c->idx_unstable, c->xm[o], c->vf[o], c->aux[o], c->key[o], c->acc_tmp, c->dyn_list, c->dyn_count,
+                               zero_dst, zero_head, zero_n4, c->scan_err, bl);
+        else
+            hipLaunchKernelGGL(k_stable_scatter_fast<false>, dim3(nb + bl.nblocks), dim3(TPB), bl.lds_bytes, c->stream, d, old_end, c->rank_off,
+                               head, c->idx_unstable, c->xm[o], c->vf[o], c->aux[o], c->key[o], c->acc_tmp, c->dyn_list, c->dyn_count,
+                               zero_dst, zero_head, zero_n4, c->scan_err, bl);
+        SPH_LAUNCH_CHECK(c);
+        c->next_heads_zero = true;
+        c->sort_fast_pending = false;
+        c->n_sort_fast = (c->n_sort_fast + 1) & 0x7fffffff;
+        return sort_scatter_done(c, o, zero_ix, sort_acc, bl.nblocks > 0, bl_key);
     }
     CellIdx16 off_ix;
     int* off_out = nullptr;
@@ -236,13 +418,6 @@
         hipLaunchKernelGGL(k_stable_scatter<false>, dim3(nb + bl.nblocks), dim3(TPB), bl.lds_bytes, c->stream, d, c->idx_unstable, c->xm[o],
                            c->vf[o], c->aux[o], c->key[o], c->acc_tmp, c->dyn_list, c->dyn_count, zero_dst, zero_n4, bl);
     SPH_LAUNCH_CHECK(c);
-    c->next_cells_zero = true;
-    c->cur = o;
-    sphd_sorted(c->dv, bl.nblocks > 0, bl_key);
-    if (sort_acc) {
-        float4* t = c->acc;
-        c->acc = c->acc_tmp;
-        c->acc_tmp = t;
-    }
-    return 0;
-}
+    c->n_sort_general = (c->n_sort_general + 1) & 0x7fffffff;
+    return sort_scatter_done(c, o, zero_ix, sort_acc, bl.nblocks > 0, bl_key);
+}
```
